# the-byte-bender/GraphAudio

Hardware: AMD Instinct MI355X
Metric: rendered frames/sec @48kHz, 1024-voice convolver graph (higher is better)
Workload: dtype f32

## Files before the change

### graphaudio_amd/csrc/ga_api.cpp

```cpp
#include <algorithm>
#include <cstring>

#include <execinfo.h>
#include <signal.h>
#include <unistd.h>

#include "ga_engine.hpp"

using namespace ga;

static void ga_segv_handler(int sig) {
  void* frames[64];
  int n = backtrace(frames, 64);
  const char msg[] = "\n[graphaudio_hip] fatal signal, native backtrace:\n";
  (void)!write(2, msg, sizeof(msg) - 1);
  backtrace_symbols_fd(frames, n, 2);
  signal(sig, SIG_DFL);
  raise(sig);
}
__attribute__((constructor)) static void ga_install_handler() {
  const char* e = getenv("GA_BACKTRACE");
  if (e && e[0] == '1') signal(SIGSEGV, ga_segv_handler);
}

struct ga_context {
  Context c;
  explicit ga_context(int sr) : c(sr) {}
};

namespace {
template <class F>
int guardRO(ga_context* h, F&& f) {
  if (!h) return GA_ERR_INVALID_ARGUMENT;
  try {
    f(h->c);
    return GA_OK;
  } catch (const Err& e) {
    h->c.lastError = e.msg;
    return e.code;
  } catch (const std::bad_alloc&) {
    h->c.lastError = "out of host memory";
    return GA_ERR_OUT_OF_MEMORY;
  } catch (const std::exception& e) {
    h->c.lastError = e.what();
    return GA_ERR_INVALID_OPERATION;
  } catch (...) {
    h->c.lastError = "unknown error";
    return GA_ERR_INVALID_OPERATION;
  }
}
template <class F>
int guard(ga_context* h, F&& f) {
  if (h) h->c.apiEpoch++;
  return guardRO(h, std::forward<F>(f));
}
NodeS* typed(Context& c, int id, int type) {
  NodeS* n = c.node(id);
  if (n->type != type) fail(GA_ERR_INVALID_ARGUMENT, "node has the wrong type for this call");
  return n;
}
float clampf(float v, float mn, float mx) {
  if (v < mn) return mn;
  if (v > mx) return mx;
  return v;
}
void addEvent(ParamS& p, const ParamEvent& e) {
  size_t lo = 0, hi = p.events.size();
  while (lo < hi) {
    size_t mid = (lo + hi) >> 1;
    if (e.time < p.events[mid].time) hi = mid; else lo = mid + 1;
  }
  p.events.insert(p.events.begin() + lo, e);
}
ParamS makeParam(float def, float mn, float mx, bool arate) {
  ParamS p;
  p.def = def;
  p.minv = mn;
  p.maxv = mx;
  p.arate = arate;
  p.value = def;
  return p;
}
}

int64_t Context::chunkLimit(int64_t) {
    int64_t limit = maxChunkBlocks;
    {
      size_t freeB = 0, totalB = 0;
      if (hipMemGetInfo(&freeB, &totalB) == hipSuccess) {
        double perBlock = 0, fixedBytes = 0;
        int convRowsMax = 0;
        for (auto& g : groups) convRowsMax = std::max(convRowsMax, (int)((g->rows.size() + 127) / 128 * 128));
        perBlock += (double)convRowsMax * kBins * 4.0 * 4.0;
        for (auto& np : nodes)
          if (np->type == GA_NODE_CONVOLVER && np->ir && np->convPath == 4)
          {
            perBlock += (double)((np->isTrueStereo ? 2 : np->ir->nch) + (np->isTrueStereo ? 4 : np->ir->nch)) * 1024.0;
            const double inCh = np->isTrueStereo ? 2 : np->ir->nch, slots = np->isTrueStereo ? 4 : np->ir->nch;
            fixedBytes += (inCh * (np->ir->coarseP + 1) + slots * (double)kCoarseMaxP) * 65536.0;
          }
          else if (np->type == GA_NODE_CONVOLVER && np->ir && np->convPath != 1)
            perBlock += (double)(np->ir->nch + 2 * (np->isTrueStereo ? 2 : np->ir->nch)) * kBins * 8.0;
        perBlock += ((double)nodes.size() * 2.0 + 64.0) * kBlock * 4.0;
        double budget = ((double)freeB + (double)slabBlocks.size() * (double)((size_t)1 << 30) * 0.0) * memBudgetFraction;
        budget += (double)(planes[0].bytes + planes[1].bytes + planes[2].bytes + planes[3].bytes);
        budget += (double)(planesB[0].bytes + planesB[1].bytes + planesB[2].bytes + planesB[3].bytes + planesBalt[0].bytes + planesBalt[1].bytes);
        budget += (double)slabAll.size() * (double)slabFrames * 4.0;
        budget += (double)(coarseX.bytes + coarseY.bytes + coarseM.bytes);
        int64_t byMem = (int64_t)(std::max(budget - fixedBytes, 0.0) / std::max(perBlock, 1.0));
        limit = std::max<int64_t>(1, std::min<int64_t>(limit, byMem));
      }
    }
  return limit;
}

void Context::processBlocks(float* const* outPlanar, float* outInterleaved, int channels, int64_t blockCount, bool deviceOut) {
  if (blockCount < 0) fail(GA_ERR_OUT_OF_RANGE, "blockCount");
  if (disposed) fail(GA_ERR_DISPOSED, "context disposed");
  flushHandOver();
  if (outInterleaved || outPlanar == nullptr) {
    if (channels < 1 || channels > 32) fail(GA_ERR_OUT_OF_RANGE, "channels");
    if (!outInterleaved) fail(GA_ERR_INVALID_ARGUMENT, "Buffer too small for interleaved output.");
  } else if (channels < 0 || channels > 32) {
    fail(GA_ERR_OUT_OF_RANGE, "channels");
  }
  GA_HIP(hipSetDevice(device));
  const hipMemcpyKind kind = deviceOut ? hipMemcpyDeviceToDevice : hipMemcpyDeviceToHost;
  int64_t doneBlocks = 0;
  while (doneBlocks < blockCount) {
    int64_t nblk = std::min(blockCount - doneBlocks, chunkLimit(blockCount - doneBlocks));
    runChunk(nblk, nullptr);
    const int64_t done = chunkBlocksDone;
    if (done <= 0) fail(GA_ERR_INVALID_OPERATION, "render made no progress");
    const int64_t base = doneBlocks * kBlock;
    if (outInterleaved) {
      float* stage = outInterleaved + base * channels;
// ... 10 lines not shown
        stage = ilvDev;
      }
      for (const SegCh& sg : chunkSegCh) {
        InterleaveSrc src{};
        const int used = std::min(channels, sg.ch);
        for (int ch = 0; ch < used; ch++) src.ch[ch] = busSlabs[ch];
        launch_interleave(stream, stage, src, channels, used, sg.b0 * kBlock, (sg.b1 - sg.b0) * kBlock);
      }
      if (!deviceOut)
        GA_HIP(hipMemcpyAsync(outInterleaved + base * channels, ilvDev, (size_t)done * kBlock * channels * sizeof(float), kind, stream));
    } else {
      for (const SegCh& sg : chunkSegCh) {
        const int used = std::min(channels, sg.ch);
        for (int ch = 0; ch < used; ch++)
          if (outPlanar[ch])
            GA_HIP(hipMemcpyAsync(outPlanar[ch] + base + sg.b0 * kBlock, busSlabs[ch] + sg.b0 * kBlock,
                                  sizeof(float) * (size_t)(sg.b1 - sg.b0) * kBlock, kind, stream));
      }
    }
    GA_HIP(hipStreamSynchronize(stream));
    doneBlocks += done;
  }
  stats.device_bytes_in_use = devBytes;
}

void Context::render(float* const* out, int channels, int64_t frameCount, int64_t startIndex, bool deviceOut) {
  if (channels == 0 || !out) fail(GA_ERR_INVALID_ARGUMENT, "Output buffer must have at least one channel.");
  if (frameCount <= 0) fail(GA_ERR_OUT_OF_RANGE, "Frame count must be positive.");
  if (startIndex < 0) fail(GA_ERR_OUT_OF_RANGE, "Start index must be non-negative.");
  if (channels < 0 || channels > 32) fail(GA_ERR_OUT_OF_RANGE, "channelIndex");
  for (int ch = 0; ch < channels; ch++)
    if (!out[ch]) fail(GA_ERR_INVALID_ARGUMENT, "Channel buffer is null.");
  if (disposed) fail(GA_ERR_DISPOSED, "context disposed");
  GA_HIP(hipSetDevice(device));
  const hipMemcpyKind kind = deviceOut ? hipMemcpyDeviceToDevice : hipMemcpyDeviceToHost;
  struct Pipelined {
    Context& c;
    const bool callerAsync;
    explicit Pipelined(Context& cc) : c(cc), callerAsync(cc.asyncMode) { c.asyncMode = true; }
    ~Pipelined() { c.asyncMode = callerAsync; }
  } pipelined(*this);
  struct Drain {
    Context& c;
    const bool blocking;
    ~Drain() {
      if (blocking && c.stream) (void)hipStreamSynchronize(c.stream);
      if (blocking && c.copyStream) (void)hipStreamSynchronize(c.copyStream);
    }
  } drain{*this, !pipelined.callerAsync};
  int64_t written = 0;
  if (cachedFrames > 0) {
    if (channels > cachedCh) fail(GA_ERR_OUT_OF_RANGE, "channelIndex");
    int toCopy = (int)std::min<int64_t>(cachedFrames, frameCount);
    for (int ch = 0; ch < channels; ch++)
      GA_HIP(hipMemcpyAsync(out[ch] + startIndex, cacheDev + (size_t)ch * kBlock + (kBlock - cachedFrames), sizeof(float) * toCopy,
                            kind, stream));
    if (!asyncMode) GA_HIP(hipStreamSynchronize(stream));
    written = toCopy;
    cachedFrames -= toCopy;
  }
  while (written < frameCount) {
    int64_t need = frameCount - written;
    int64_t nblk = (need + kBlock - 1) / kBlock;
    const int64_t limit = chunkLimit(nblk);
    nblk = std::min(nblk, limit);
    bool direct = (deviceOut || hostDirect) && need >= nblk * kBlock;
    float* tgt[32];
    for (int ch = 0; ch < channels && direct; ch++) {
      float* p = out[ch] + startIndex + written;
      if (!deviceOut) {
        hipPointerAttribute_t at{};
        if (hipPointerGetAttributes(&at, p) != hipSuccess || at.type != hipMemoryTypeHost || !at.devicePointer) {
          (void)hipGetLastError();
          direct = false;
          break;
        }
        p = (float*)at.devicePointer;
      }
      tgt[ch] = p;
      direct = (((uintptr_t)p) & 15) == 0;
    }
    struct Target {
      Context& c;
      ~Target() { std::memset(c.busTarget, 0, sizeof(c.busTarget)); }
    } target{*this};
    const bool defer = direct && !deviceOut && pipelined.callerAsync && hostDefer && ownStream;
    if (defer) {
      const size_t rowBytes = ((size_t)nblk * kBlock * sizeof(float) + 255) & ~(size_t)255;
      if (deferStageBytes < rowBytes * 32) {
        flushHandOver();
        if (deferStage) {
          GA_HIP(hipStreamSynchronize(stream));
          dfree(deferStage, deferStageBytes);
        }
        deferStageBytes = rowBytes * 32;
        deferStage = (float*)dalloc(deferStageBytes);
      }
      for (int ch = 0; ch < channels; ch++) busTarget[ch] = (float*)((char*)deferStage + (size_t)ch * (deferStageBytes / 32));
    } else if (direct) {
      for (int ch = 0; ch < channels; ch++) busTarget[ch] = tgt[ch];
    }
    runChunk(nblk, nullptr);
    if (defer)
      for (int ch = 0; ch < channels; ch++)
        pendingHandOver.push_back(HandOver{busTarget[ch], tgt[ch], out[ch] + startIndex + written, chunkBlocksDone * kBlock});
    std::memset(busTarget, 0, sizeof(busTarget));
    const int64_t done = chunkBlocksDone;
    if (done <= 0) fail(GA_ERR_INVALID_OPERATION, "render made no progress");
    if (channels > chunkMinDestCh) fail(GA_ERR_OUT_OF_RANGE, "channelIndex");
    const int64_t chunkFrames = done * kBlock;
    const int64_t toCopy = std::min(chunkFrames, need);
    if (direct) {
    } else if (!deviceOut && ownStream && pipelined.callerAsync && hostCopyStream) {
      handOverToHost(busSlabs.data(), out, channels, startIndex + written, toCopy);
    } else {
      for (int ch = 0; ch < channels; ch++)
        GA_HIP(hipMemcpyAsync(out[ch] + startIndex + written, busSlabs[ch], sizeof(float) * toCopy, kind, stream));
    }
    const int64_t excess = chunkFrames - toCopy;
    if (excess > 0) {
      cachedCh = chunkMinDestCh;
      for (int ch = 0; ch < cachedCh; ch++)
        GA_HIP(hipMemcpyAsync(cacheDev + (size_t)ch * kBlock, busSlabs[ch] + chunkFrames - kBlock, sizeof(float) * kBlock,
                              hipMemcpyDeviceToDevice, stream));
      cachedFrames = (int)excess;
    }
    if (!asyncMode) GA_HIP(hipStreamSynchronize(stream));
    written += toCopy;
  }
  if (!pipelined.callerAsync) {
    GA_HIP(hipStreamSynchronize(stream));
    harvestProfile(true);
  }
  stats.device_bytes_in_use = devBytes;
}

extern "C" {

const char* ga_strerror(int code) {
  switch (code) {
    case GA_OK: return "ok";
    case GA_ERR_INVALID_ARGUMENT: return "invalid argument";
    case GA_ERR_OUT_OF_RANGE: return "argument out of range";
    case GA_ERR_INVALID_OPERATION: return "invalid operation";
    case GA_ERR_DISPOSED: return "object disposed";
    case GA_ERR_CYCLE: return "audio graph cycle detected";
    case GA_ERR_UNSUPPORTED: return "unsupported on the device path";
    case GA_ERR_DEVICE: return "HIP device error";
    case GA_ERR_OUT_OF_MEMORY: return "out of memory";
    case GA_ERR_NO_DEVICE: return "no HIP device";
    default: return "unknown error code";
  }
}
const char* ga_version(void) { return "graphaudio-hip 0.1 (gfx950)"; }
int ga_device_count(void) {
  int n = 0;
  if (hipGetDeviceCount(&n) != hipSuccess) return 0;
  return n;
}

int ga_context_create(int sample_rate, int device_ordinal, ga_context** out) {
  if (!out) return GA_ERR_INVALID_ARGUMENT;
  if (sample_rate <= 0) return GA_ERR_OUT_OF_RANGE;
  ga_context* h = nullptr;
  try {
    h = new ga_context(sample_rate);
    h->c.init_device(device_ordinal);
    auto d = std::make_unique<NodeS>();
    d->id = 0;
    d->type = GA_NODE_DESTINATION;
    d->inputs.resize(1);
    d->inputs[0].channelCount = 2;
    h->c.nodes.push_back(std::move(d));
    *out = h;
    return GA_OK;
  } catch (const Err& e) {
    delete h;
    return e.code;
  } catch (...) {
    delete h;
    return GA_ERR_DEVICE;
  }
}
int ga_context_destroy(ga_context* ctx) {
  delete ctx;
  return GA_OK;
}
const char* ga_last_error(ga_context* ctx) { return ctx ? ctx->c.lastError.c_str() : ""; }
double ga_current_time(ga_context* ctx) { return ctx ? ctx->c.currentTime : 0.0; }
int64_t ga_current_block(ga_context* ctx) { return ctx ? ctx->c.currentBlock : 0; }
int ga_set_option(ga_context* ctx, const char* key, double value) {
  return guard(ctx, [&](Context& c) {
    std::string k = key ? key : "";
    if (k == "max_chunk_blocks") c.maxChunkBlocks = std::max<int64_t>(1, std::min<int64_t>(32768, (int64_t)value));
    else if (k == "profile") c.profile = value != 0;
    else if (k == "profile_every") c.profileEvery = (int)std::max<int64_t>(1, value);
    else if (k == "time_fft") c.useTimeFft = value != 0;
    else if (k == "fft64") c.fft64 = value != 0;
    else if (k == "tconv_radix16") c.useRadix16 = value != 0;
    else if (k == "async") {
      if (c.asyncMode && value == 0) c.synchronize();
      c.asyncMode = value != 0;
    }
    else if (k == "coarse") c.useCoarse = value != 0;
    else if (k == "coarse_overlap") c.coarseOverlap = value != 0;
    else if (k == "coarse_carry") c.coarseCarry = value != 0;
    else if (k == "coarse_tail") c.coarseTail = value != 0;
    else if (k == "coarse_tail_private") c.coarseTailPrivate = value != 0;
    else if (k == "sim_replay") c.simReplay = value != 0;
    else if (k == "twin_channels") c.twinChannels = value != 0;
    else if (k == "cycle_delay_split") c.cycleDelaySplit = value != 0;
    else if (k == "resample_fast") c.resampleFast = value != 0;
    else if (k == "rate_mod_walk") c.rateModWalk = value != 0;
    else if (k == "conv_reference_order") c.convRefOrder = (int)std::min(2.0, std::max(0.0, value));
    else if (k == "conv_ref_min_deviation") c.convRefMinDeviation = std::max(0.0, value);
    else if (k == "coarse_premix") c.coarsePremix = value != 0;
    else if (k == "coarse_ext_history") c.coarseExtHist = value != 0;
    else if (k == "coarse_wide") c.coarseWide = value != 0;
    else if (k == "gain_pass_through") c.gainPassThrough = value != 0;
    else if (k == "gain_fold") c.gainFold = value != 0;
    else if (k == "coarse_mfma") c.coarseMfma = value != 0;
    else if (k == "biquad_time_split") c.biquadTimeSplit = (int)std::min(2.0, std::max(0.0, value));
    else if (k == "biquad_split_max_deviation") c.biquadSplitMaxDeviation = std::max(0.0, value);
    else if (k == "biquad_split_min_frames") c.biquadSplitMinFrames = std::max<int64_t>(2048, (int64_t)value);
    else if (k == "host_direct") c.hostDirect = value != 0;
    else if (k == "host_defer") c.hostDefer = value != 0;
    else if (k == "table_upload_kernel") c.tableUploadKernel = value != 0;
    else if (k == "comm_timeout_s") c.commTimeoutS = std::max(1.0, value);
    else if (k == "host_copy_stream") c.hostCopyStream = value != 0;
    else if (k == "coarse_min_blocks") c.coarseMinBlocks = std::max<int64_t>(1, (int64_t)value);
    else if (k == "debug_tconv_n2") c.debugTconvN2 = (int)value;
    else if (k == "mem_budget_fraction") c.memBudgetFraction = std::min(0.95, std::max(0.05, value));
    else fail(GA_ERR_INVALID_ARGUMENT, "unknown option " + k);
  });
}
int ga_get_stats(ga_context* ctx, ga_stats* out) {
  return guardRO(ctx, [&](Context& c) {
    if (!out) fail(GA_ERR_INVALID_ARGUMENT, "null pointer");
    c.harvestProfile(true);
    c.stats.device_bytes_in_use = c.devBytes;
    c.stats.n_nodes = (int)c.nodes.size();
    int rows = 0;
    for (auto& g : c.groups) rows += (int)g->rows.size();
    c.stats.n_conv_rows = rows;
    *out = c.stats;
  });
}
int ga_synchronize(ga_context* ctx) {
  return guardRO(ctx, [&](Context& c) { c.synchronize(); });
}
int ga_context_set_stream(ga_context* ctx, void* hip_stream) {
  return guard(ctx, [&](Context& c) {
    c.flushHandOver();
    GA_HIP(hipStreamSynchronize(c.stream));
    c.waitHostCopies();
    if (c.ownStream && c.stream) (void)hipStreamDestroy(c.stream);
    c.stream = (hipStream_t)hip_stream;
    c.ownStream = false;
  });
}

int ga_buffer_create(ga_context* ctx, const float* const* planar, int channels, int64_t frames, int sample_rate, int* out_id) {
  return guard(ctx, [&](Context& c) {
    if (!planar || !out_id) fail(GA_ERR_INVALID_ARGUMENT, "null pointer");
    if (channels < 1 || channels > 32) fail(GA_ERR_OUT_OF_RANGE, "Channel count must be between 1 and 32");
    if (frames < 0) fail(GA_ERR_OUT_OF_RANGE, "Length must be non-negative");
    if (sample_rate <= 0) fail(GA_ERR_OUT_OF_RANGE, "Sample rate must be positive");
    auto b = std::make_unique<PlayBuf>();
    b->channels = channels;
    b->length = frames;
    b->sampleRate = sample_rate;
    b->stride = (frames + 8 + 63) / 64 * 64;
    b->host.resize(channels);
    GA_HIP(hipSetDevice(c.device));
    size_t bytes = (size_t)b->stride * channels * sizeof(float);
    b->dev = c.dallocSkewed(bytes, &b->devBase, &b->devBytes);
    GA_HIP(hipMemsetAsync(b->dev, 0, bytes, c.stream));
    for (int i = 0; i < channels; i++) {
      if (!planar[i]) fail(GA_ERR_INVALID_ARGUMENT, "null channel pointer");
      b->host[i].assign(planar[i], planar[i] + frames);
      if (frames)
        GA_HIP(hipMemcpyAsync(b->dev + (size_t)i * b->stride, planar[i], sizeof(float) * frames, hipMemcpyHostToDevice, c.stream));
    }
    GA_HIP(hipStreamSynchronize(c.stream));
    c.buffers.push_back(std::move(b));
    c.bufVersion++;
    *out_id = (int)c.buffers.size() - 1;
  });
}
int ga_buffer_release(ga_context* ctx, int buffer_id) {
  return guard(ctx, [&](Context& c) {
    PlayBuf* b = c.buffer(buffer_id);
    if (!b || b->released) return;
    b->released = true;
    c.releasedPending.push_back(buffer_id);
  });
}

int ga_node_create(ga_context* ctx, int node_type, int* out_id) {
// ... 487 lines not shown
```

### graphaudio_amd/csrc/ga_chunk.cpp

```cpp
#include "ga_chunk_internal.hpp"

namespace ga {

float* getSlab(Context& c) {
  if (c.slabFree.empty()) {
    size_t slabBytes = (size_t)c.slabFrames * sizeof(float);
    size_t count = std::max<size_t>(8, std::min<size_t>(1024, ((size_t)1 << 30) / slabBytes));
    char* blk = (char*)c.dalloc(slabBytes * count);
    c.slabBlocks.push_back(blk);
    for (size_t i = 0; i < count; i++) {
      float* p = (float*)(blk + i * slabBytes);
      c.slabAll.push_back(p);
      c.slabFree.push_back(p);
    }
  }
  float* p = c.slabFree.back();
  c.slabFree.pop_back();
  return p;
}

void resetSlabs(Context& c, int64_t frames) {
  int64_t need = roundup(frames, 256);
  if (need > c.slabFrames) {
    GA_HIP(hipStreamSynchronize(c.stream));
// ... 508 lines not shown
  Context& c_ = *this; (void)c_;
  std::vector<int>& topo = r.topo;
  int& maxDepth = r.maxDepth; int& maxLevel = r.maxLevel; (void)maxDepth; (void)maxLevel;
  int64_t& n = r.n; (void)n;
  std::vector<double>& bt = r.bt; (void)bt;
  std::vector<int>& srcIds = r.srcIds; (void)srcIds;
  std::vector<SrcPlanOut>& srcPlans = r.srcPlans; (void)srcPlans;
  std::vector<Segment>& segs = r.segs; (void)segs;
  const int64_t frames = r.n * kBlock; (void)frames;
  int& bHistMax = r.bHistMax; (void)bHistMax;
  for (int id : topo) {
    NodeS& nd = *nodes[id];
    if (nd.type != GA_NODE_DELAY) continue;
    nd.delayLoaded = false;
    int rings = std::max(nd.delayRings, 2);
    for (const Segment& sg : segs)
      for (const NodeSeg& ns : sg.nodes)
        if (ns.id == id) rings = std::max(rings, ns.ins[0].bufCh);
    nd.delayRings = rings;
    const size_t maxD = (size_t)nd.maxDelaySamples;
    if (nd.delayHistRings < rings) {
      float* nh = (float*)dalloc(maxD * rings * sizeof(float));
      GA_HIP(hipMemsetAsync(nh, 0, maxD * rings * sizeof(float), stream));
      if (nd.delayHist) {
        GA_HIP(hipMemcpyAsync(nh, nd.delayHist, maxD * nd.delayHistRings * sizeof(float), hipMemcpyDeviceToDevice, stream));
        GA_HIP(hipStreamSynchronize(stream));
        dfree(nd.delayHist, maxD * nd.delayHistRings * sizeof(float));
      }
      nd.delayHist = nh;
      nd.delayHistRings = rings;
    }
    const int64_t cap = roundup(frames, 4096);
    if (nd.delayCap < cap || nd.delayLineRings < rings) {
      if (nd.delayLine) {
        GA_HIP(hipStreamSynchronize(stream));
        dfree(nd.delayLine, (maxD + (size_t)nd.delayCap) * nd.delayLineRings * sizeof(float));
      }
      nd.delayCap = std::max(nd.delayCap, cap);
      nd.delayLineRings = rings;
      nd.delayLine = (float*)dalloc((maxD + (size_t)nd.delayCap) * rings * sizeof(float));
    }
    nd.delayW.assign(rings, 0);
    nd.delayR.assign(rings, 0);
  }

  if (r.stage != 2) resetSlabs(*this, frames);
  if (zerosLen < frames) {
    if (zeros) {
      GA_HIP(hipStreamSynchronize(stream));
      dfree(zeros, (size_t)zerosLen * 4);
    }
    zerosLen = roundup(frames, 4096);
    zeros = (float*)dalloc((size_t)zerosLen * 4);
    GA_HIP(hipMemsetAsync(zeros, 0, (size_t)zerosLen * 4, stream));
  }
  if (busCapFrames < frames) {
    GA_HIP(hipStreamSynchronize(stream));
    for (float* p : busSlabs) dfree(p, (size_t)busCapFrames * 4);
    busSlabs.clear();
    busCapFrames = roundup(frames, 4096);
  }
  while ((int)busSlabs.size() < 32 && (int)busSlabs.size() < std::max(destOutCh, 2)) busSlabs.push_back((float*)dalloc((size_t)busCapFrames * 4));
  {
    int mx = 0;
    for (auto& sg : segs)
      if (r.stage != 1) mx = std::max(mx, sg.nodes.back().outCh);
    while ((int)busSlabs.size() < mx) busSlabs.push_back((float*)dalloc((size_t)busCapFrames * 4));
  }

}

void Context::chunkExecute(ChunkRun& r) {
  Context& c_ = *this; (void)c_;
  int& maxDepth = r.maxDepth; int& maxLevel = r.maxLevel; (void)maxDepth; (void)maxLevel;
  int64_t& n = r.n; (void)n;
  std::vector<double>& bt = r.bt; (void)bt;
  std::vector<int>& srcIds = r.srcIds; (void)srcIds;
  std::vector<SrcPlanOut>& srcPlans = r.srcPlans; (void)srcPlans;
  std::vector<Segment>& segs = r.segs; (void)segs;
  const int64_t frames = r.n * kBlock; (void)frames;
  int& bHistMax = r.bHistMax; (void)bHistMax;
  Exec& ex = *r.ex;
  r.tmPlan = nowMs();
  if (!pendingHandOver.empty()) {
    std::vector<HandOver> hv;
    hv.swap(pendingHandOver);
    hipStream_t st = stream;
    ex.plan.launches.insert(ex.plan.launches.begin(), Plan::L{[hv, st](uint8_t*) {
      for (const HandOver& h : hv) GA_HIP(hipMemcpyAsync(h.dst_host, h.src, sizeof(float) * (size_t)h.n, hipMemcpyDeviceToHost, st));
    }, LK_OTHER, 0.0, 0.0});
  }
  ex.trajOffFinal = ex.plan.putv(ex.traj);
  size_t tbytes = ex.plan.host.size();
  const int slot = asyncMode ? (int)(chunkSeq & 1) : 0;
  void*& thost = slot ? tablesHostB : tablesHost;
  size_t& thostBytes = slot ? tablesHostBBytes : tablesHostBytes;
  if (asyncMode && chunkDone[slot]) GA_HIP(hipEventSynchronize(chunkDone[slot]));
  if (thostBytes < tbytes) {
    if (thost) {
      GA_HIP(hipStreamSynchronize(stream));
      (void)hipHostFree(thost);
    }
    thostBytes = (tbytes + tbytes / 4 + 4096 + 15) & ~(size_t)15;
    GA_HIP(hipHostMalloc(&thost, thostBytes, hipHostMallocDefault));
  }
  ensure(tables, std::max(tablesHostBytes, tablesHostBBytes));
  std::memcpy(thost, ex.plan.host.data(), tbytes);
  if (tableUploadKernel) launch_table_upload(stream, tables.p, thost, tbytes);
  else GA_HIP(hipMemcpyAsync(tables.p, thost, tbytes, hipMemcpyHostToDevice, stream));
  uint8_t* base = (uint8_t*)tables.p;

  std::vector<std::pair<hipEvent_t, hipEvent_t>> evs;
  std::vector<int> evKind;
  std::vector<double> evBytes;
  hipEvent_t evBegin = nullptr, evEnd = nullptr;
  const bool profile = profileNow;
  if (profile) {
    GA_HIP(hipEventCreate(&evBegin));
    GA_HIP(hipEventCreate(&evEnd));
    GA_HIP(hipEventRecord(evBegin, stream));
  }
  for (auto& l : ex.plan.launches) {
    hipEvent_t e0 = nullptr, e1 = nullptr;
    if (profile) {
      GA_HIP(hipEventCreate(&e0));
      GA_HIP(hipEventCreate(&e1));
      GA_HIP(hipEventRecord(e0, stream));
    }
    l.fn(base);
    if (profile) {
      GA_HIP(hipEventRecord(e1, stream));
      evs.push_back({e0, e1});
      evKind.push_back(l.kind);
      evBytes.push_back(l.bytes);
    }
    if (l.kind == GA_STAGE_COARSE_SECTION) continue;
    stats.kernel_launches++;
    if (l.kind >= 0 && l.kind < 16) {
      stats.stage_launches[l.kind]++;
      stats.stage_bytes[l.kind] += l.bytes;
      stats.stage_flops[l.kind] += l.flops;
    }
  }
  for (auto& x : extraProf) {
    evs.push_back({x.e0, x.e1});
    evKind.push_back(x.kind);
    evBytes.push_back(x.bytes);
  }
  extraProf.clear();
  if (profile) GA_HIP(hipEventRecord(evEnd, stream));
  GA_HIP(hipGetLastError());
  r.tmLaunch = nowMs();
  if (profileNow) pendingProf.push_back(ProfBatch{evBegin, evEnd, std::move(evs), std::move(evKind), std::move(evBytes)});
  if (asyncMode) {
    if (!chunkDone[slot]) GA_HIP(hipEventCreateWithFlags(&chunkDone[slot], hipEventDisableTiming));
    GA_HIP(hipEventRecord(chunkDone[slot], stream));
    harvestProfile(false);
  } else {
    GA_HIP(hipStreamSynchronize(stream));
    harvestProfile(true);
  }
  chunkSeq++;
  if (gaTiming)
    fprintf(stderr, "[ga]   host detail: topo %.2f, sources %.2f, sim %.2f | resources %.2f, params %.2f, exec %.2f ms\n", r.tmTopo - r.tm0,
            r.tmSrc - r.tmTopo, r.tmSim - r.tmSrc, r.tmRes - r.tmSim, r.tmPre - r.tmRes, r.tmPlan - r.tmPre);
  if (gaTiming)
    fprintf(stderr, "[ga] chunk %lld blocks: sim %.2f ms, plan %.2f ms, enqueue %.2f ms, wait %.2f ms\n", (long long)n, r.tmSim - r.tm0,
            r.tmPlan - r.tmSim, r.tmLaunch - r.tmPlan, nowMs() - r.tmLaunch);

}

void Context::chunkCommit(ChunkRun& r) {
  Context& c_ = *this; (void)c_;
  int& maxDepth = r.maxDepth; int& maxLevel = r.maxLevel; (void)maxDepth; (void)maxLevel;
  int64_t& n = r.n; (void)n;
  std::vector<double>& bt = r.bt; (void)bt;
  std::vector<int>& srcIds = r.srcIds; (void)srcIds;
  std::vector<SrcPlanOut>& srcPlans = r.srcPlans; (void)srcPlans;
  std::vector<Segment>& segs = r.segs; (void)segs;
  const int64_t frames = r.n * kBlock; (void)frames;
  int& bHistMax = r.bHistMax; (void)bHistMax;
  for (size_t i = 0; i < srcIds.size(); i++) {
    NodeS& s = *nodes[srcIds[i]];
    SrcPlanOut& po = srcPlans[i];
    if (s.type != GA_NODE_BUFFER_SOURCE) {
      if (po.gone && po.goneAt <= n) {
        if (!s.endedRaised) endedQueue.push_back(srcIds[i]);
        s.endedRaised = true;
        if (po.goneAt == n) pending.push_back([this, id = srcIds[i]]() { doDispose(id); });
      }
      continue;
    }
    if (s.spans.empty()) continue;
    int64_t firstPlay = -1;
    for (const SrcSpan& sp : s.spans)
      if ((sp.phase == SRC_PLAY || sp.phase == SRC_END) && firstPlay < 0) firstPlay = sp.b0;
    if (firstPlay < 0 || firstPlay >= n) continue;
    int64_t lastProcessed = n;
    if (po.gone && po.goneAt <= n) lastProcessed = po.goneAt;
    int64_t played = lastProcessed - firstPlay;
    PlayBuf* pb = s.bufId >= 0 ? buffers[s.bufId].get() : nullptr;
    bool rate1 = true;
    if (pb) rate1 = sourceGeom(*this, s, *pb).effectiveRate == 1.0;
    if (s.gsr && s.gsrWalked >= 0) {
      if (played == s.gsrWalked) {
        s.playbackPosition = s.gsrTail.pp;
        for (int k = 0; k < 4; k++) s.gsrW[k] = s.gsrTail.w[k];
        s.gsrPos = s.gsrTail.pos;
        s.gsrReady = s.gsrTail.ready;
      } else if (!(po.gone && po.goneAt <= n)) {
        fail(GA_ERR_DEVICE, "internal: a walked source ends its chunk at another block than its walk");
      }
    } else if (s.gsr) {
      if (!s.gsrBlocks.empty()) {
        const GsrBlock& e = s.gsrBlocks[std::min<size_t>((size_t)played, s.gsrBlocks.size() - 1)];
        s.playbackPosition = e.pp;
        for (int k = 0; k < 4; k++) s.gsrW[k] = e.w[k];
        s.gsrPos = e.pos;
        s.gsrReady = e.ready;
      }
    } else if (rate1) {
      s.playbackPosition += played * kBlock;
      if (s.loop && pb) {
        SrcGeom g = sourceGeom(*this, s, *pb);
        int64_t len = g.loopEndFrame - g.loopStartFrame;
        if (s.playbackPosition >= g.loopEndFrame && len > 0)
          s.playbackPosition = g.loopStartFrame + ((s.playbackPosition - g.loopEndFrame) % len);
      }
    } else {
      s.rsBlocks += played;
    }
    if (po.reachedEnd && po.endBlock < n) {
      s.stopTime = bt[po.endBlock + 1];
      s.hasStopped = true;
    }
    if (po.gone && po.goneAt <= n) {
      if (!s.endedRaised) endedQueue.push_back(srcIds[i]);
      s.endedRaised = true;
      if (po.goneAt == n) pending.push_back([this, id = srcIds[i]]() { doDispose(id); });
    }
  }
  for (int id : r.streamIds) streamReplay(*nodes[id], n, bt, true);
  if (r.stage == 1) return;
  currentBlock += n;
  currentTime = bt[n];
  stats.blocks_rendered = currentBlock;
  stats.chunks++;
  stats.segments += (int64_t)segs.size();
  chunkBlocksDone = n;
  chunkSegCh.clear();
  for (const Segment& sg : segs) chunkSegCh.push_back(SegCh{sg.b0, sg.b1, sg.nodes.back().outCh});
}

void Context::runChunkImpl(int64_t nblocks, float* const* ) {
  ChunkRun r;
  r.n = nblocks;
  r.tm0 = nowMs();
  GA_HIP(hipSetDevice(device));
  if (disposed) fail(GA_ERR_DISPOSED, "context disposed");
  drain();
  if (!releasedPending.empty() || ++chunksSinceGc >= 64) collectGarbage();
  latched = true;
  profileNow = profile && (profileSeq++ % std::max(profileEvery, 1)) == 0;
  chunkTopology(r);
  if (!r.rateMods.empty()) {
    runTwoStageChunk(r);
    return;
  }
  chunkSimulate(r);
  chunkResources(r);
  r.tmRes = nowMs();
  bqSplitUsed = 0;
  r.ex = std::make_unique<Exec>(*this, r.n, r.segs);
  r.ex->outViews.resize(r.segs.size());
  r.ex->plan.host.resize(16);
  chunkStaleSeed(r);
  chunkParamCurves(r);
  const double tmPar = nowMs();
  chunkConvScratch(r);
  r.tmPre = nowMs();
  double tmNodes = 0, tmConv = 0;
  for (int d = 0; d <= r.maxDepth; d++) {
    const double a = nowMs();
    chunkPlanNodes(r, d);
    const double b = nowMs();
    chunkPlanConvolvers(r, d);
    tmNodes += b - a;
    tmConv += nowMs() - b;
  }
  chunkDelayCommit(r);
  chunkStaleCommit(r);
  chunkExecute(r);
  const double tmEx = nowMs();
  chunkCommit(r);
  chunkRetire(r);
  if (gaTiming)
    fprintf(stderr, "[ga]   host detail: param curves %.3f, conv scratch %.3f, plan nodes %.3f, plan convolvers %.3f, commit %.3f ms\n",
            tmPar - r.tmRes, r.tmPre - tmPar, tmNodes, tmConv, nowMs() - tmEx);
}

void Context::chunkRetire(ChunkRun& r) {
  if (!r.ex->outViews.empty() && !r.segs.empty()) {
    if (!lastViews.empty() && viewsPool.size() < 8) viewsPool.push_back(std::move(lastViews));
    lastViews = std::move(r.ex->outViews.back());
    r.ex->outViews.pop_back();
    const size_t sl = r.segs.size() - 1;
    if (sl < r.ex->outScale.size() && !r.ex->outScale[sl].empty()) lastViewScale = r.ex->outScale[sl];
    else lastViewScale.clear();
    if (sl < r.ex->outCurve.size() && !r.ex->outCurve[sl].empty()) lastViewCurve = r.ex->outCurve[sl];
    else lastViewCurve.clear();
    lastViewFrames = r.n * kBlock;
    lastViewSlabGen = slabGen;
  }
  for (auto& ov : r.ex->outViews)
    if (!ov.empty() && viewsPool.size() < 8) viewsPool.push_back(std::move(ov));
  if (!r.segs.empty() && simReplay) {
    if (lastSegNodes.capacity() && segNodePool.size() < 8) {
      lastSegNodes.clear();
      segNodePool.push_back(std::move(lastSegNodes));
    }
    lastSegNodes = std::move(r.segs.back().nodes);
    lastSegHash = r.segs.back().hash;
    lastSegEpoch = apiEpoch;
    lastSegGraphVersion = graphVersion;
    r.segs.pop_back();
  }
  for (Segment& sg : r.segs) {
    sg.nodes.clear();
    if (segNodePool.size() < 8) segNodePool.push_back(std::move(sg.nodes));
  }
  r.ex.reset();
}

void Context::runTwoStageChunk(ChunkRun& r) {
  ChunkRun r1;
  r1.stage = 1;
  r1.n = r.n;
  r1.tm0 = r.tm0;
  r1.maxDepth = r.maxDepth;
  r1.maxLevel = r.maxLevel;
  r1.rateMods = r.rateMods;
  r1.coneRoots = std::move(r.coneRoots);
// ... 176 lines not shown
```

### graphaudio_amd/csrc/ga_chunk_internal.hpp

```cpp
#pragma once
#include <time.h>

#include <algorithm>
#include <array>
#include <cstdio>
#include <cstdlib>
#include <cstring>
#include <unordered_map>

#include "ga_engine.hpp"

namespace ga {

static inline uint64_t hmix(uint64_t h, uint64_t v) {
  h ^= v + 0x9e3779b97f4a7c15ull + (h << 6) + (h >> 2);
  return h;
}

static inline int64_t roundup(int64_t v, int64_t m) { return (v + m - 1) / m * m; }

struct Plan {
  std::vector<uint8_t> host;
  struct L {
    std::function<void(uint8_t*)> fn;
// ... 351 lines not shown
        if (!n_.delayAudible && timelineOnly) {
          const ParamS& pd = n_.params[0];
          const double t0 = (*blockTimes)[brel], dts = 1.0 / c.sampleRate;
          bool pending = false;
          for (int r = 0; r < ch && !n_.delayAudible; r++) {
            auto& m = model[r];
            for (auto& run : m.runs)
              if (run.second == OPEN || run.second + maxD >= m.pos) pending = true;
            if (m.runs.empty()) continue;
            for (int i = 0; i < kBlock && !n_.delayAudible; i++) {
              const float dtv = param_value_at(pd.events.data(), (int)pd.events.size(), pd.value, pd.arate ? t0 + i * dts : t0);
              int d = (int)(dtv * (float)c.sampleRate);
              d = std::min(std::max(d, 0), maxD);
              if (d == 0) continue;
              const int64_t q = m.pos + i - d;
              for (auto& run : m.runs)
                if (q >= run.first && (run.second == OPEN || q < run.second)) {
                  n_.delayAudible = true;
                  break;
                }
            }
          }
          if (!n_.delayAudible && pending && extraBreaks) extraBreaks->push_back(brel + 1);
        } else if (!n_.delayAudible && dmax > 0) {
          dmin = std::max(dmin, 1);
          int64_t nextFlip = OPEN;
          for (int r = 0; r < ch && !n_.delayAudible; r++) {
            auto& m = model[r];
            const int64_t lo = m.pos - dmax, hi = m.pos + (kBlock - 1) - dmin;
            for (auto& run : m.runs) {
              const int64_t rs = run.first, re = run.second == OPEN ? OPEN : run.second - 1;
              if (rs <= hi && re >= lo) {
                n_.delayAudible = true;
                break;
              }
              if (rs > hi) {
                int64_t k = (rs + dmin - (kBlock - 1) - m.pos + kBlock - 1) / kBlock;
                nextFlip = std::min(nextFlip, B + std::max<int64_t>(k, 1));
              }
            }
          }
          if (!n_.delayAudible && nextFlip != OPEN && extraBreaks) extraBreaks->push_back(nextFlip - c.currentBlock);
        }
        ns.delayAudible = n_.delayAudible;
        n_.outputs[0].bufCh = ch;
        n_.outputs[0].silent = !n_.delayAudible;
        break;
      }
      default: fail(GA_ERR_UNSUPPORTED, "node type not supported on the device path");
    }
    if (!n_.outputs.empty()) {
      ns.outCh = n_.outputs[0].bufCh;
      ns.outSilent = n_.outputs[0].silent;
      ns.outZero = !n_.outputs[0].silent && n_.outputs[0].zero;
    }
  }

  uint64_t hashSeg(const Segment& s) {
    uint64_t h = 1469598103934665603ull;
    for (const NodeSeg& ns : s.nodes) {
      h = hmix(h, (uint64_t)ns.id);
      h = hmix(h, ((uint64_t)ns.outCh << 8) | (ns.outSilent ? 1 : 0) | ((uint64_t)ns.srcPhase << 4) | (ns.bqActive ? 2 : 0) |
                      ((uint64_t)ns.outMask << 16) | ((uint64_t)ns.panMode << 48) | ((uint64_t)(ns.panDyn ? 1 : 0) << 52) |
                      ((uint64_t)(ns.outZero ? 1 : 0) << 53));
      for (const InSeg& is : ns.ins) {
        h = hmix(h, ((uint64_t)is.bufCh << 1) | (is.silent ? 1 : 0));
        for (const TermS& t : is.terms) h = hmix(h, ((uint64_t)t.node << 16) | ((uint64_t)t.out << 8) | (uint64_t)t.ch | ((uint64_t)t.stale << 60));
      }
      for (const InSeg& is : ns.pins)
        for (const TermS& t : is.terms) h = hmix(h, 0x5151ull ^ (((uint64_t)t.node << 16) | ((uint64_t)t.out << 8) | (uint64_t)t.ch | ((uint64_t)t.stale << 60)));
    }
    for (const InSeg& is : s.probe) {
      h = hmix(h, 0x7070ull ^ (is.silent ? 1 : 0));
      for (const TermS& t : is.terms) h = hmix(h, ((uint64_t)t.node << 16) | ((uint64_t)t.out << 8) | (uint64_t)t.ch);
    }
    return h;
  }
};

struct Exec {
  Context& c;
  int64_t n, frames;
  Plan plan;
  std::vector<Segment>& segs;
  std::unordered_map<uint64_t, float*> nodeSlab, inSlab;
  std::vector<float*> nodeSlab01;
  std::vector<std::vector<Views>> outViews;
  std::vector<const float*> terms;
  std::vector<float> termGains;
  bool anyTermGain = false;
  std::vector<std::vector<float>> outScale;
  float scaleOf(int si, int node) const { return (si < (int)outScale.size() && !outScale[si].empty()) ? outScale[si][node] : 1.f; }
  void setScale(int si, int node, float g) {
    if ((int)outScale.size() <= si) outScale.resize(si + 1);
    if (outScale[si].empty()) outScale[si].assign(c.nodes.size(), 1.f);
    outScale[si][node] = g;
  }
  std::vector<const float*> termCurves;
  bool anyTermCurve = false;
  std::vector<std::vector<const float*>> outCurve;
  const float* curveOf(int si, int node) const { return (si < (int)outCurve.size() && !outCurve[si].empty()) ? outCurve[si][node] : nullptr; }
  void setCurve(int si, int node, const float* cv) {
    if ((int)outCurve.size() <= si) outCurve.resize(si + 1);
    if (outCurve[si].empty()) outCurve[si].assign(c.nodes.size(), nullptr);
    outCurve[si][node] = cv;
  }
  void pushTerm(const float* p, float g, const float* cv = nullptr) {
    termGains.resize(terms.size(), 1.f);
    termCurves.resize(terms.size(), nullptr);
    terms.push_back(p);
    termGains.push_back(g);
    termCurves.push_back(cv);
    if (g != 1.f) anyTermGain = true;
    if (cv) anyTermGain = anyTermCurve = true;
  }
  std::vector<MixJob> mixJobs;
  std::vector<DownmixJob> dmJobs;
  std::vector<GainJob> gainJobs;
  std::vector<BiquadJob> bqJobs[kMaxBiquadSections + 1];
  std::vector<BiquadSection> bqSecs;
  std::vector<BiquadScanJob> bqScans[kMaxBiquadSections + 1];
  std::vector<const std::vector<float>*> bqMats[kMaxBiquadSections + 1];
  int bqG = 0;
  int64_t bqK = 0;
  size_t bqZeroFrom = 0;
  std::vector<BiquadDynJob> bqDynJobs;
  std::vector<LoopJob> loopJobs;
  std::vector<ResampleJob> rsJobs;
  std::vector<ResampleFastJob> rsFastJobs;
  std::vector<GsrJob> gsrJobs;
  std::vector<StreamJob> streamJobs;
  std::vector<ConstJob> constJobs;
  std::vector<OscJob> oscJobs;
  std::vector<PanJob> panJobs;
  std::vector<DelayJob> delayJobs;
  std::vector<PanDynJob> panDynJobs;
  std::vector<ParamModJob> pmodJobs;
  std::vector<ResampleBlock> traj;
  bool mixAligned = true;
  struct ConvInRow {
    Views* p = nullptr;
    size_t n = 0;
    bool empty() const { return n == 0; }
    size_t size() const { return n; }
    Views& operator[](size_t i) const { return p[i]; }
  };
  struct ConvIn {
    std::vector<int> slot;
    std::vector<Views> flat;
    size_t nsegs = 1, used = 0;
    bool has(int id) const { return id < (int)slot.size() && slot[id] >= 0; }
    ConvInRow operator[](int id) {
      if (id >= (int)slot.size()) slot.resize(id + 1, -1);
      if (slot[id] < 0) {
        slot[id] = (int)used++;
        if (flat.size() < used * nsegs) flat.resize(std::max(used * nsegs, 2 * flat.size()));
      }
      return ConvInRow{flat.data() + (size_t)slot[id] * nsegs, nsegs};
    }
  } convIn;

  Exec(Context& c_, int64_t n_, std::vector<Segment>& s) : c(c_), n(n_), frames(n_ * kBlock), segs(s) {
    nodeSlab01.assign(c.nodes.size() * 2, nullptr);
    convIn.slot.assign(c.nodes.size(), -1);
    convIn.nsegs = std::max<size_t>(segs.size(), 1);
  }
// ... 521 lines not shown
```

### graphaudio_amd/csrc/ga_coarse.hip

```cpp
#include "ga_kernels.hpp"
#include "ga_fft16.hpp"

#include <hip/hip_runtime.h>

#include <algorithm>
#include <atomic>
#include <string>
#include <type_traits>
#include <utility>
#include <cstdio>
#include <cstdlib>

namespace ga {

struct LdsLimit {
  std::atomic<uint64_t> done{0};
  void raise(const void* kern, size_t need, const char* what) {
    int dev = 0;
    (void)hipGetDevice(&dev);
    const uint64_t bit = 1ull << (dev & 63);
    if (done.load(std::memory_order_relaxed) & bit) return;
    if (hipFuncSetAttribute(kern, hipFuncAttributeMaxDynamicSharedMemorySize, 160 * 1024) == hipSuccess) {
      done.fetch_or(bit);
      return;
// ... 995 lines not shown
        acc[w].add(x);
      }
    }
  }
}
__global__ __launch_bounds__(64 * kPremixWaves) void coarse_premix_kernel(const PremixJob* __restrict jobs, const PremixTerm* __restrict terms) {
  __shared__ v4f part[kPremixWaves - 1][2][kPremixWords][64];
  const PremixJob J = jobs[blockIdx.y];
  if (J.flags & 4) {
    if (blockIdx.x >= (unsigned)kPremixCopyWgs) return;
    const GA_GLOBAL v4f* src = (const GA_GLOBAL v4f*)terms[J.term0].in;
    GA_GLOBAL v4f* dst = (GA_GLOBAL v4f*)J.out;
    const int64_t nw = J.n / 4, step = (int64_t)kPremixCopyWgs * blockDim.x * 2;
    for (int64_t i = (int64_t)blockIdx.x * blockDim.x * 2 + threadIdx.x; i < nw; i += step) {
      const int64_t i2 = i + blockDim.x;
      const v4f a = src[i], b = i2 < nw ? src[i2] : a;
      dst[i] = a;
      if (i2 < nw) dst[i2] = b;
    }
    return;
  }
  const int64_t tile0 = (int64_t)blockIdx.x * kPremixTile;
  if (tile0 >= J.n) return;
  const int lane = threadIdx.x & 63, wv = __builtin_amdgcn_readfirstlane(threadIdx.x >> 6);
  int64_t f[kPremixWords];
  bool live[kPremixWords], keep[kPremixWords];
  uint32_t off[kPremixWords], coff[kPremixWords];
  Kahan4 acc[kPremixWords];
#pragma unroll
  for (int w = 0; w < kPremixWords; w++) {
    f[w] = tile0 + (int64_t)(w * 64 + lane) * 4;
    live[w] = f[w] < J.n;
    keep[w] = live[w] && f[w] >= J.carry_from;
    off[w] = live[w] ? (uint32_t)(f[w] * 4) : 0u;
    coff[w] = (uint32_t)((f[w] - J.carry_from) * 4);
    acc[w] = Kahan4{v4f{0.f, 0.f, 0.f, 0.f}, v4f{0.f, 0.f, 0.f, 0.f}};
  }
  const int per = ((J.nterms + kPremixWaves - 1) / kPremixWaves + kPremixAhead - 1) / kPremixAhead * kPremixAhead;
  const int t0 = min(J.nterms, wv * per), t1 = min(J.nterms, t0 + per);
  const bool carry_here = (J.flags & 2) && tile0 + kPremixTile > J.carry_from;
  if (J.flags & 1) {
    if (carry_here) premix_stream<true, true>(J, terms, t0, t1, lane, off, keep, coff, acc);
    else premix_stream<true, false>(J, terms, t0, t1, lane, off, keep, coff, acc);
  } else {
    if (carry_here) premix_stream<false, true>(J, terms, t0, t1, lane, off, keep, coff, acc);
    else premix_stream<false, false>(J, terms, t0, t1, lane, off, keep, coff, acc);
  }
  if (wv > 0) {
#pragma unroll
    for (int w = 0; w < kPremixWords; w++) {
      part[wv - 1][0][w][lane] = acc[w].s;
      part[wv - 1][1][w][lane] = acc[w].c;
    }
  }
  __syncthreads();
  if (wv == 0) {
#pragma unroll
    for (int w = 0; w < kPremixWords; w++) {
#pragma unroll
      for (int q = 0; q < kPremixWaves - 1; q++) {
        acc[w].add(part[q][0][w][lane]);
        acc[w].add(-part[q][1][w][lane]);
      }
      if (live[w]) stg4(J.out + f[w], acc[w].s);
    }
  }
}
const char* launch_coarse_premix(hipStream_t s, const PremixJob* jobs_dev, int njobs, const PremixTerm* terms_dev, int64_t max_n) {
  if (njobs <= 0 || max_n <= 0) return "";
  const int64_t gx = (max_n + kPremixTile - 1) / kPremixTile;
  if (gx > 0x7fffffff || max_n >= ((int64_t)1 << 29)) launch_fail("coarse pre-mix: chunk too long");
  for (int j0 = 0; j0 < njobs; j0 += 32768)
    hipLaunchKernelGGL(coarse_premix_kernel, dim3((unsigned)gx, std::min(32768, njobs - j0)), dim3(64 * kPremixWaves), 0, s, jobs_dev + j0, terms_dev);
  return "coarse_premix_kernel";
}

void launch_coarse_hist(hipStream_t s, const CoarseHistJob* jobs_dev, int njobs, int64_t max_len) {
  if (njobs <= 0 || max_len <= 0) return;
  const int gx = (int)std::min<int64_t>((max_len / 4 + 255) / 256, 64);
  for (int j0 = 0; j0 < njobs; j0 += 32768)
    hipLaunchKernelGGL(coarse_hist_kernel, dim3(gx, std::min(32768, njobs - j0)), dim3(256), 0, s, jobs_dev + j0);
}

__global__ __launch_bounds__(256) void table_upload_kernel(v4f* __restrict dst, const v4f* __restrict src, size_t n16) {
  for (size_t i = (size_t)blockIdx.x * 256 + threadIdx.x; i < n16; i += (size_t)gridDim.x * 256) ((GA_GLOBAL v4f*)dst)[i] = ((const GA_GLOBAL v4f*)src)[i];
}
void launch_table_upload(hipStream_t s, void* dst, const void* src_pinned, size_t bytes) {
  const size_t n16 = (bytes + 15) / 16;
  if (!n16) return;
  const unsigned grid = (unsigned)std::min<size_t>((n16 + 255) / 256, 64);
  hipLaunchKernelGGL(table_upload_kernel, dim3(grid), dim3(256), 0, s, (v4f*)dst, (const v4f*)src_pinned, n16);
}

}
```

### graphaudio_amd/csrc/ga_comm.cpp

```cpp
#include <dlfcn.h>

#include <cstring>
#include <mutex>

#include <chrono>
#include <thread>

#include "ga_engine.hpp"

#if __has_include(<rccl/rccl.h>)
#include <rccl/rccl.h>
static_assert(NCCL_UNIQUE_ID_BYTES == GA_COMM_ID_BYTES, "include/graphaudio_hip.h: GA_COMM_ID_BYTES != NCCL_UNIQUE_ID_BYTES");
static_assert(sizeof(ncclUniqueId) == GA_COMM_ID_BYTES, "ncclUniqueId is passed by value as GA_COMM_ID_BYTES bytes");
static_assert((int)ncclSuccess == 0 && (int)ncclInProgress == 7, "restated ncclResult_t values");
static_assert((int)ncclFloat32 == 7 && (int)ncclSum == 0, "restated ncclDataType_t / ncclRedOp_t values");
#endif

namespace ga {

namespace {
constexpr int kNcclSuccess = 0, kNcclInProgress = 7, kNcclFloat32 = 7, kNcclSum = 0;
struct UniqueId {
  char internal[GA_COMM_ID_BYTES];
};
// ... 108 lines not shown
    if (r.CommGetAsyncError && r.CommGetAsyncError(comm, &async) == kNcclSuccess && async != kNcclSuccess && async != kNcclInProgress) {
      const std::string what = r.GetErrorString ? r.GetErrorString(async) : "RCCL error";
      commAbort();
      fail(GA_ERR_DEVICE, "the communicator failed (a peer rank aborted or died): " + what);
    }
    if (std::chrono::duration<double>(std::chrono::steady_clock::now() - t0).count() > commTimeoutS) {
      commAbort();
      fail(GA_ERR_DEVICE, "timed out waiting for the sharded render's collective (option comm_timeout_s)");
    }
    std::this_thread::sleep_for(std::chrono::microseconds(200));
  }
}

void Context::commDestroy() {
  if (comm) {
    try {
      if (stream) commWait();
    } catch (...) {
    }
  }
  if (comm) {
    Rccl& r = rccl();
    if (r.CommDestroy) (void)r.CommDestroy(comm);
    comm = nullptr;
  }
  commDead = false;
  commRanks = 0;
  commRank = 0;
  if (reduceBuf) {
    dfree(reduceBuf, reduceBytes);
    reduceBuf = nullptr;
    reduceBytes = 0;
  }
}

void Context::renderReduce(float* const* out, int channels, int64_t frames, int64_t start, int root) {
  if (commRanks < 1) fail(GA_ERR_INVALID_OPERATION, "ga_comm_init has not been called on this context");
  if (commDead) fail(GA_ERR_INVALID_OPERATION, "the communicator was aborted after an error; ga_comm_destroy and ga_comm_init again");
  if (root < 0 || root >= commRanks) fail(GA_ERR_OUT_OF_RANGE, "root");
  if (channels < 1 || channels > 32) fail(GA_ERR_OUT_OF_RANGE, "channelIndex");
  if (frames <= 0) fail(GA_ERR_OUT_OF_RANGE, "Frame count must be positive.");
  if (start < 0) fail(GA_ERR_OUT_OF_RANGE, "Start index must be non-negative.");
  const bool isRoot = commRank == root;
  if (isRoot) {
    if (!out) fail(GA_ERR_INVALID_ARGUMENT, "Output buffer must have at least one channel.");
    for (int ch = 0; ch < channels; ch++)
      if (!out[ch]) fail(GA_ERR_INVALID_ARGUMENT, "Channel buffer is null.");
  }
  GA_HIP(hipSetDevice(device));
  const size_t need_ = (size_t)channels * (size_t)frames * sizeof(float);
  if (reduceBytes < need_) {
    flushHandOver();
    if (reduceBuf) {
      GA_HIP(hipStreamSynchronize(stream));
      dfree(reduceBuf, reduceBytes);
    }
    reduceBytes = need_ + need_ / 8;
    reduceBuf = (float*)dalloc(reduceBytes);
  }
  float* rows[32];
  for (int ch = 0; ch < channels; ch++) rows[ch] = reduceBuf + (size_t)ch * frames;
  const bool callerAsync = asyncMode;
  asyncMode = true;
  try {
    render(rows, channels, frames, 0, true);
    if (comm) {
      Rccl& r = rccl();
      check(r, r.Reduce(reduceBuf, reduceBuf, (size_t)channels * frames, kNcclFloat32, kNcclSum, root, comm, stream), "ncclReduce");
    }
    if (isRoot) {
      float* devAlias[32];
      bool locked = callerAsync && hostDefer && ownStream && (frames % 4) == 0;
      for (int ch = 0; ch < channels && locked; ch++) {
        hipPointerAttribute_t at{};
        if (hipPointerGetAttributes(&at, out[ch] + start) != hipSuccess || at.type != hipMemoryTypeHost || !at.devicePointer ||
            (((uintptr_t)at.devicePointer) & 15)) {
          (void)hipGetLastError();
          locked = false;
        } else {
          devAlias[ch] = (float*)at.devicePointer;
        }
      }
      if (locked) {
        for (int ch = 0; ch < channels; ch++) pendingHandOver.push_back(HandOver{rows[ch], devAlias[ch], out[ch] + start, frames});
      } else if (callerAsync && ownStream && hostCopyStream) {
        handOverToHost(rows, out, channels, start, frames);
      } else {
        for (int ch = 0; ch < channels; ch++)
          GA_HIP(hipMemcpyAsync(out[ch] + start, rows[ch], (size_t)frames * sizeof(float), hipMemcpyDeviceToHost, stream));
      }
    }
  } catch (...) {
    asyncMode = callerAsync;
    commAbort();
    throw;
  }
  asyncMode = callerAsync;
  if (!callerAsync) {
    flushHandOver();
    commWait();
    harvestProfile(true);
  }
}

}
```

### graphaudio_amd/csrc/ga_engine.cpp

```cpp
#include "ga_engine.hpp"

#include <algorithm>
#include <cstdio>
#include <cstring>

namespace ga {

void launch_fail(const char* what) { fail(GA_ERR_INVALID_OPERATION, std::string("internal: ") + what); }

void* Context::dalloc(size_t bytes) {
  void* p = nullptr;
  if (bytes == 0) bytes = 256;
  GA_HIP(hipMalloc(&p, bytes));
  devBytes += (int64_t)bytes;
  return p;
}
float* Context::dallocSkewed(size_t bytes, void** base, size_t* total) {
  *total = bytes + 64 * 1024;
  *base = dalloc(*total);
  return (float*)((char*)*base + (size_t)(skewSeq++ % 64) * 1024);
}
double Context::biquadDeviation(const float* coefs, int nsec) {
  std::vector<float> key(coefs, coefs + 5 * nsec);
  uint64_t h = 1469598103934665603ull;
// ... 111 lines not shown
  float* p = (float*)((char*)bqSplitBlocks[blk] + bqSplitUsed % kBqSplitBlock);
  bqSplitUsed += bytes;
  return p;
}
int Context::persistentBuffer(const float* p, int64_t n) {
  if (!p || n <= 0) return -1;
  if (bufSpansVersion != bufVersion) {
    bufSpans.clear();
    for (size_t i = 0; i < buffers.size(); i++)
      if (buffers[i] && buffers[i]->dev) bufSpans.push_back(BufSpan{buffers[i]->dev, buffers[i]->dev + (size_t)buffers[i]->stride * buffers[i]->channels, (int)i});
    std::sort(bufSpans.begin(), bufSpans.end(), [](const BufSpan& a, const BufSpan& b) { return a.lo < b.lo; });
    bufSpansVersion = bufVersion;
  }
  auto it = std::upper_bound(bufSpans.begin(), bufSpans.end(), p, [](const float* q, const BufSpan& s) { return q < s.lo; });
  if (it == bufSpans.begin()) return -1;
  --it;
  return (p >= it->lo && p + n <= it->hi) ? it->id : -1;
}
void Context::dfree(void* p, size_t bytes) {
  if (!p) return;
  (void)hipFree(p);
  devBytes -= (int64_t)(bytes == 0 ? 256 : bytes);
}
void Context::ensure(DevArena& a, size_t bytes) {
  if (a.bytes >= bytes) return;
  if (a.p) {
    GA_HIP(hipStreamSynchronize(stream));
    dfree(a.p, a.bytes);
    a.p = nullptr;
    a.bytes = 0;
  }
  size_t nb = bytes + bytes / 8;
  a.p = dalloc(nb);
  a.bytes = nb;
  GA_HIP(hipMemsetAsync(a.p, 0, nb, stream));
}

void Context::init_device(int dev) {
  int count = 0;
  if (hipGetDeviceCount(&count) != hipSuccess || count <= 0)
    fail(GA_ERR_NO_DEVICE, "no HIP device visible: libgraphaudio_hip has no CPU fallback");
  if (dev < 0 || dev >= count) fail(GA_ERR_INVALID_ARGUMENT, "device ordinal out of range");
  device = dev;
  GA_HIP(hipSetDevice(dev));
  GA_HIP(hipStreamCreateWithFlags(&stream, hipStreamNonBlocking));
  ownStream = true;
  const double pi = 3.14159265358979323846264338327950288;
  std::vector<double2> t128(64), t256(129);
  for (int j = 0; j < 64; j++) t128[j] = make_double2(std::cos(2.0 * pi * j / 128.0), -std::sin(2.0 * pi * j / 128.0));
  for (int k = 0; k <= 128; k++) t256[k] = make_double2(std::cos(2.0 * pi * k / 256.0), -std::sin(2.0 * pi * k / 256.0));
  w128 = (double2*)dalloc(sizeof(double2) * 64);
  w256 = (double2*)dalloc(sizeof(double2) * 129);
  GA_HIP(hipMemcpy(w128, t128.data(), sizeof(double2) * 64, hipMemcpyHostToDevice));
  GA_HIP(hipMemcpy(w256, t256.data(), sizeof(double2) * 129, hipMemcpyHostToDevice));
  cacheDev = (float*)dalloc(sizeof(float) * 32 * kBlock);
}

Context::~Context() {
  if (stream) (void)hipStreamSynchronize(stream);
  try {
    commDestroy();
  } catch (...) {
  }
  for (auto& b : buffers)
    if (b && b->devBase) (void)hipFree(b->devBase);
  for (auto& g : groups) {
    if (g->histR) (void)hipFree(g->histR);
    if (g->histI) (void)hipFree(g->histI);
    if (g->overlap[0]) (void)hipFree(g->overlap[0]);
    if (g->overlap[1]) (void)hipFree(g->overlap[1]);
  }
  for (auto& a : planes)
    if (a.p) (void)hipFree(a.p);
  for (auto& a : planesB)
    if (a.p) (void)hipFree(a.p);
  for (auto& a : planesBalt)
    if (a.p) (void)hipFree(a.p);
  for (auto& np : nodes) {
    if (np && np->bHistR) (void)hipFree(np->bHistR);
    if (np && np->bHistI) (void)hipFree(np->bHistI);
    if (np && np->bOverlap) (void)hipFree(np->bOverlap);
    if (np && np->dHistBase[0]) (void)hipFree(np->dHistBase[0]);
    if (np && np->dHistBase[1]) (void)hipFree(np->dHistBase[1]);
    if (np && np->dTail[0]) (void)hipFree(np->dTail[0]);
    if (np && np->dTail[1]) (void)hipFree(np->dTail[1]);
    if (np && np->stWin[0]) (void)hipFree(np->stWin[0]);
    if (np && np->stWin[1]) (void)hipFree(np->stWin[1]);
    if (np && np->delayHist) (void)hipFree(np->delayHist);
    if (np && np->delayLine) (void)hipFree(np->delayLine);
    if (np && np->oscPhase) (void)hipFree(np->oscPhase);
    if (np && np->panDev) (void)hipFree(np->panDev);
  }
  for (auto& kv : tw16) (void)hipFree(kv.second);
  if (rateModDev) (void)hipFree(rateModDev);
  if (rateModHost) (void)hipHostFree(rateModHost);
  if (coarseTw) (void)hipFree(coarseTw);
  if (tw16pw) (void)hipFree(tw16pw);
  if (copyStream) {
    (void)hipStreamSynchronize(copyStream);
    (void)hipStreamDestroy(copyStream);
    for (int k = 0; k < 2; k++) {
      if (outReady[k]) (void)hipEventDestroy(outReady[k]);
      if (outCopied[k]) (void)hipEventDestroy(outCopied[k]);
      if (outStage[k]) (void)hipFree(outStage[k]);
    }
  }
  if (stream2) {
    (void)hipStreamSynchronize(stream2);
    (void)hipStreamDestroy(stream2);
    for (auto& e : dGroupEv)
      if (e) (void)hipEventDestroy(e);
    if (dJoinEv) (void)hipEventDestroy(dJoinEv);
  }
  for (auto& x : extraProf) { (void)hipEventDestroy(x.e0); (void)hipEventDestroy(x.e1); }
  if (coarseX.p) (void)hipFree(coarseX.p);
  if (coarseY.p) (void)hipFree(coarseY.p);
  if (coarseM.p) (void)hipFree(coarseM.p);
  if (deferStage) (void)hipFree(deferStage);
  for (auto& r : retired) (void)hipFree(r.first);
  for (auto& kv : resamplers)
    if (kv.second->devSamples) (void)hipFree(kv.second->devSamples);
  for (auto& np : nodes)
    if (np && np->staleBuf) {
      (void)hipFree(np->staleBuf);
      (void)hipFree(np->staleNext);
    }
  for (float* p : bqSplitBlocks) (void)hipFree(p);
  if (ilvDev) (void)hipFree(ilvDev);
  if (tables.p) (void)hipFree(tables.p);
  if (tablesHost) (void)hipHostFree(tablesHost);
  if (tablesHostB) (void)hipHostFree(tablesHostB);
  for (auto& e : chunkDone)
    if (e) (void)hipEventDestroy(e);
  for (auto& b : pendingProf) {
    (void)hipEventDestroy(b.begin);
    (void)hipEventDestroy(b.end);
    for (auto& e : b.evs) { (void)hipEventDestroy(e.first); (void)hipEventDestroy(e.second); }
  }
  for (void* p : slabBlocks) (void)hipFree(p);
  for (void* p : bqBlocks) (void)hipFree(p);
  for (float* p : busSlabs) (void)hipFree(p);
  if (zeros) (void)hipFree(zeros);
  if (w128) (void)hipFree(w128);
  if (w256) (void)hipFree(w256);
  for (auto& kv : twC) (void)hipFree(kv.second);
  if (cacheDev) (void)hipFree(cacheDev);
  if (stream && ownStream) (void)hipStreamDestroy(stream);
}

void Context::executeOrPost(std::function<void()> cmd) {
  if (disposed) fail(GA_ERR_DISPOSED, "context disposed");
  if (latched && !inRender) cmd(); else pending.push_back(std::move(cmd));
}
void Context::post(std::function<void()> cmd) {
  if (disposed) fail(GA_ERR_DISPOSED, "context disposed");
  pending.push_back(std::move(cmd));
}
void Context::drain() {
  while (!pending.empty()) {
    auto cmd = std::move(pending.front());
    pending.pop_front();
    apiEpoch++;
    try {
      cmd();
    } catch (const Err&) {
    }
  }
}

NodeS* Context::node(int id) {
  if (id < 0 || id >= (int)nodes.size()) fail(GA_ERR_INVALID_ARGUMENT, "bad node id");
  return nodes[id].get();
}
ParamS* Context::param(int nid, int p) {
  NodeS* n = node(nid);
  if (p < 0 || p >= (int)n->params.size()) fail(GA_ERR_INVALID_ARGUMENT, "bad param index");
  return &n->params[p];
}
PlayBuf* Context::buffer(int id) {
  if (id < 0) return nullptr;
  if (id >= (int)buffers.size() || !buffers[id]) fail(GA_ERR_INVALID_ARGUMENT, "bad buffer id");
  return buffers[id].get();
}
void Context::collectGarbage() {
  chunksSinceGc = 0;
  if (!releasedPending.empty()) {
    std::vector<char> used(buffers.size(), 0);
    for (auto& np : nodes) {
      if (!np || np->disposed) continue;
      if (np->bufId >= 0 && np->bufId < (int)used.size()) used[np->bufId] = 1;
      if (np->irBuf >= 0 && np->irBuf < (int)used.size()) used[np->irBuf] = 1;
      for (auto& e : np->dHistExt)
        if (e.first && e.second >= 0 && e.second < (int)used.size()) used[e.second] = 1;
      if (np->type == GA_NODE_STREAM_SOURCE) {
        if (np->stCurrent >= 0 && np->stCurrent < (int)used.size()) used[np->stCurrent] = 1;
        for (int id : np->stQueued) if (id >= 0 && id < (int)used.size()) used[id] = 1;
        for (int id : np->stProcessed) if (id >= 0 && id < (int)used.size()) used[id] = 1;
      }
    }
    std::vector<int> keep;
    bool synced = false;
    for (int id : releasedPending) {
      if (id < 0 || id >= (int)buffers.size() || !buffers[id]) continue;
      if (used[id]) {
        keep.push_back(id);
        continue;
      }
      if (!synced && stream) {
        (void)hipStreamSynchronize(stream);
        synced = true;
      }
      PlayBuf& b = *buffers[id];
      if (b.devBase) dfree(b.devBase, b.devBytes);
      bufVersion++;
      for (auto it = irCache.begin(); it != irCache.end();)
        it = it->first.first == id ? irCache.erase(it) : std::next(it);
      buffers[id].reset();
    }
    releasedPending.swap(keep);
  }
  for (auto it = irCache.begin(); it != irCache.end();) {
    if (it->second.use_count() == 1) {
      if (stream) (void)hipStreamSynchronize(stream);
      it = irCache.erase(it);
    } else {
      ++it;
    }
  }
}

InputS* Context::inputOf(const InRef& r) {
  NodeS* n = nodes[r.node].get();
  if (r.input >= 0) return &n->inputs[r.input];
  return nullptr;
}

void Context::harvestProfile(bool wait) {
  while (!pendingProf.empty()) {
    ProfBatch& b = pendingProf.front();
    if (wait) GA_HIP(hipEventSynchronize(b.end));
    else if (hipEventQuery(b.end) != hipSuccess) { (void)hipGetLastError(); break; }
    float ms = 0;
    GA_HIP(hipEventElapsedTime(&ms, b.begin, b.end));
    stats.device_ms_total += ms;
    stats.profiled_chunks++;
    for (size_t i = 0; i < b.evs.size(); i++) {
      GA_HIP(hipEventElapsedTime(&ms, b.evs[i].first, b.evs[i].second));
      const int k = b.kinds[i];
      if (k == LK_MAC || k == LK_CMAC) stats.mac_ms_total += ms;
      else if (k == LK_FFT || k == LK_IFFT || k == LK_CFWD || k == LK_CINV || k == LK_CHIST) stats.fft_ms_total += ms;
      else if (k != GA_STAGE_COARSE_SECTION) stats.other_ms_total += ms;
      if (k >= 0 && k < 16) stats.stage_ms[k] += ms;
      (void)hipEventDestroy(b.evs[i].first);
      (void)hipEventDestroy(b.evs[i].second);
    }
    (void)hipEventDestroy(b.begin);
    (void)hipEventDestroy(b.end);
    pendingProf.pop_front();
  }
}
void Context::flushHandOver() {
  for (const HandOver& h : pendingHandOver)
    GA_HIP(hipMemcpyAsync(h.dst_host, h.src, sizeof(float) * (size_t)h.n, hipMemcpyDeviceToHost, stream));
  pendingHandOver.clear();
}
void Context::synchronize() {
  GA_HIP(hipSetDevice(device));
  flushHandOver();
  commWait();
  waitHostCopies();
  harvestProfile(true);
  freeRetired();
}
void Context::freeRetired() {
  for (auto& r : retired) dfree(r.first, r.second);
  retired.clear();
}
void Context::waitHostCopies() {
  if (!copyStream) return;
  GA_HIP(hipStreamSynchronize(copyStream));
  outPending[0] = outPending[1] = false;
}
void Context::handOverToHost(const float* const* src, float* const* out, int channels, int64_t offset, int64_t frames) {
  if (!copyStream) {
    GA_HIP(hipStreamCreateWithFlags(&copyStream, hipStreamNonBlocking));
    for (int k = 0; k < 2; k++) {
      GA_HIP(hipEventCreateWithFlags(&outReady[k], hipEventDisableTiming));
      GA_HIP(hipEventCreateWithFlags(&outCopied[k], hipEventDisableTiming));
    }
  }
  const int k = outCur;
  outCur ^= 1;
  const size_t need = (size_t)channels * (size_t)frames * sizeof(float);
  if (outStageBytes[k] < need) {
    if (outPending[k]) GA_HIP(hipEventSynchronize(outCopied[k]));
    outPending[k] = false;
    if (outStage[k]) {
      GA_HIP(hipStreamSynchronize(stream));
      dfree(outStage[k], outStageBytes[k]);
      outStage[k] = nullptr;
      outStageBytes[k] = 0;
    }
    outStage[k] = (float*)dalloc(need);
    outStageBytes[k] = need;
  }
  if (outPending[k]) GA_HIP(hipStreamWaitEvent(stream, outCopied[k], 0));
  for (int ch = 0; ch < channels; ch++)
    GA_HIP(hipMemcpyAsync(outStage[k] + (size_t)ch * frames, src[ch], sizeof(float) * (size_t)frames, hipMemcpyDeviceToDevice, stream));
  GA_HIP(hipEventRecord(outReady[k], stream));
  GA_HIP(hipStreamWaitEvent(copyStream, outReady[k], 0));
  for (int ch = 0; ch < channels; ch++)
    GA_HIP(hipMemcpyAsync(out[ch] + offset, outStage[k] + (size_t)ch * frames, sizeof(float) * (size_t)frames, hipMemcpyDeviceToHost, copyStream));
  GA_HIP(hipEventRecord(outCopied[k], copyStream));
  outPending[k] = true;
}

void Context::connectTo(int src, int out, InRef in) {
  graphVersion++;
  if (in.node == src) fail(GA_ERR_INVALID_OPERATION, "Cannot connect a node to itself");
  OutputS& o = nodes[src]->outputs[out];
  if (std::find(o.connectedInputs.begin(), o.connectedInputs.end(), in) != o.connectedInputs.end()) return;
  o.connectedInputs.push_back(in);
  if (in.input >= 0) {
    InputS& i = nodes[in.node]->inputs[in.input];
    Conn c{src, out};
    if (std::find(i.connected.begin(), i.connected.end(), c) == i.connected.end()) {
      i.connected.push_back(c);
      i.dirty = true;
    }
  } else {
    auto& m = nodes[in.node]->params[-1 - in.input].modulation;
    std::pair<int, int> c{src, out};
    if (std::find(m.begin(), m.end(), c) == m.end()) m.push_back(c);
  }
}
static void removeFromInput(Context& c, int src, int out, InRef in) {
  if (in.input >= 0) {
    InputS& i = c.nodes[in.node]->inputs[in.input];
    Conn cc{src, out};
    auto it = std::find(i.connected.begin(), i.connected.end(), cc);
    if (it != i.connected.end()) i.connected.erase(it);
    i.dirty = true;
  } else {
    auto& m = c.nodes[in.node]->params[-1 - in.input].modulation;
// ... 11 lines not shown
    removeFromInput(*this, src, out, in);
  }
}
void Context::outputDisconnectAll(int src, int out) {
  graphVersion++;
  OutputS& o = nodes[src]->outputs[out];
  std::vector<InRef> ins = o.connectedInputs;
  o.connectedInputs.clear();
  for (const InRef& in : ins) removeFromInput(*this, src, out, in);
}
void Context::inputDisconnectAll(InRef in) {
  std::vector<Conn> outs;
  if (in.input >= 0) {
    outs = nodes[in.node]->inputs[in.input].connected;
  } else {
    for (auto& m : nodes[in.node]->params[-1 - in.input].modulation) outs.push_back(Conn{m.first, m.second});
  }
  for (const Conn& c : outs) disconnectFrom(c.node, c.out, in);
  if (in.input >= 0) nodes[in.node]->inputs[in.input].dirty = true;
}
void Context::doDispose(int id) {
  graphVersion++;
  NodeS& n = *nodes[id];
  if (n.disposed) return;
  n.disposed = true;
  for (int o = 0; o < (int)n.outputs.size(); o++) outputDisconnectAll(id, o);
  for (int i = 0; i < (int)n.inputs.size(); i++) {
    inputDisconnectAll(InRef{id, i});
    n.inputs[i].bufCh = 0;
  }
  for (int p = 0; p < (int)n.params.size(); p++) inputDisconnectAll(InRef{id, -1 - p});
  if (n.type == GA_NODE_DELAY) {
    if (stream) (void)hipStreamSynchronize(stream);
    if (n.delayHist) dfree(n.delayHist, (size_t)n.maxDelaySamples * n.delayHistRings * sizeof(float));
    if (n.delayLine) dfree(n.delayLine, ((size_t)n.maxDelaySamples + (size_t)n.delayCap) * n.delayLineRings * sizeof(float));
    n.delayHist = n.delayLine = nullptr;
    n.delayHistRings = n.delayLineRings = 0;
    n.delayCap = 0;
  }
  if (n.staleBuf) {
    if (stream) (void)hipStreamSynchronize(stream);
    dfree(n.staleBuf, (size_t)n.staleRows * kBlock * sizeof(float));
    dfree(n.staleNext, (size_t)n.staleRows * kBlock * sizeof(float));
    n.staleBuf = n.staleNext = nullptr;
    n.staleRows = 0;
  }
  if (n.type == GA_NODE_BUFFER_SOURCE) n.bufId = -1;
  if (n.type == GA_NODE_STREAM_SOURCE && n.stState != GA_STREAM_STOPPED) {
    n.stState = GA_STREAM_STOPPED;
    streamFlushToProcessed(n);
  }
  if (n.type == GA_NODE_CONVOLVER) {
    releaseConvState(n);
    n.ir.reset();
    n.irBuf = -1;
  }
}

void Context::releaseConvState(NodeS& n) {
  graphVersion++;
  for (auto& r : n.convRows)
    if (r.group) r.group->rows[r.idx] = {-1, 0};
  n.convRows.clear();
  if (n.bHistR || n.bOverlap) {
    if (stream) (void)hipStreamSynchronize(stream);
    if (n.ir) {
      size_t hb = (size_t)n.bInCh * kBins * std::max(n.ir->P - 1, 1) * sizeof(float);
      dfree(n.bHistR, hb);
      dfree(n.bHistI, hb);
    } else {
      (void)hipFree(n.bHistR);
      (void)hipFree(n.bHistI);
    }
    dfree(n.bOverlap, (size_t)n.bSlots * 2 * kBlock * sizeof(float));
  }
  if (n.dHist[0]) {
    if (stream) (void)hipStreamSynchronize(stream);
    dfree(n.dHistBase[0], n.dHistBytes);
    dfree(n.dHistBase[1], n.dHistBytes);
    n.dHistBase[0] = n.dHistBase[1] = nullptr;
  }
  if (n.dTail[0]) {
    if (stream) (void)hipStreamSynchronize(stream);
    for (int b = 0; b < 2; b++) dfree(n.dTail[b], (size_t)n.dTailLen * n.dTailCh * sizeof(float));
  }
  n.dTail[0] = n.dTail[1] = nullptr;
  n.dTailLen = 0;
  n.dTailCh = n.dTailCur = 0;
  n.dTailSig = 0;
  n.dTailSeq = ~0ull - 1;
  n.dHist[0] = n.dHist[1] = nullptr;
  n.dHistExt.clear();
  n.dHistLen = 0;
  n.dHistCur = 0;
  n.dHistZero = true;
  n.dLeader = -1;
  n.dGroupSize = 0;
  n.everFed = false;
  fusionKeyValid = false;
  n.bHistR = n.bHistI = n.bOverlap = nullptr;
  n.bHistPlane = -1;
  n.convPath = 0;
  n.bShared = true;
  n.bHistZero = true;
  n.bOvCur = 0;
}

void Context::flushPlaneHistories(int pair) {
  std::vector<HistJobB> jobs;
  int maxh = 1;
  for (int id : bResidents[pair]) {
    NodeS* n = node(id);
    if (!n || n->bHistPlane != pair || !n->ir || !n->bHistR) continue;
    const int h = n->ir->P - 1;
    const size_t hstride = (size_t)kBins * std::max(h, 1);
    for (int c = 0; c < n->bHistNx && h > 0; c++) {
      const size_t off = (size_t)(n->bHistRow + c) * kBins * n->bHistTxb + n->bHistOff;
      jobs.push_back(HistJobB{n->bHistR + c * hstride, xPlane(pair, 0) + off, h, n->bHistTxb, h, 0});
      jobs.push_back(HistJobB{n->bHistI + c * hstride, xPlane(pair, 1) + off, h, n->bHistTxb, h, 0});
    }
    maxh = std::max(maxh, h);
    n->bHistPlane = -1;
  }
  bResidents[pair].clear();
  if (jobs.empty()) return;
  HistJobB* tab = nullptr;
  GA_HIP(hipHostMalloc((void**)&tab, jobs.size() * sizeof(HistJobB), hipHostMallocDefault));
  memcpy(tab, jobs.data(), jobs.size() * sizeof(HistJobB));
  launch_hist_copy_b(stream, tab, (int)jobs.size(), maxh);
  GA_HIP(hipGetLastError());
  GA_HIP(hipStreamSynchronize(stream));
  GA_HIP(hipHostFree(tab));
}

ConvRowRef Context::addGroupRow(const std::shared_ptr<IrSpectra>& ir, int ch, int depth, int nodeId) {
  auto key = std::make_tuple(ir.get(), ch, depth);
  ConvGroup* g;
  auto it = groupOf.find(key);
  if (it == groupOf.end()) {
    auto ng = std::make_unique<ConvGroup>();
    ng->ir = ir;
    ng->irCh = ch;
    ng->depth = depth;
    ng->P = ir->P;
    g = ng.get();
    groups.push_back(std::move(ng));
    groupOf[key] = g;
  } else {
    g = it->second;
  }
  int idx = (int)g->rows.size();
  g->rows.push_back({nodeId, ch});
  if (idx < g->rp && g->histR) {
    const int hist = g->P - 1;
    if (hist > 0) {
      GA_HIP(hipMemset2DAsync(g->histR + idx, (size_t)g->rp * 4, 0, 4, (size_t)kBins * hist, stream));
      GA_HIP(hipMemset2DAsync(g->histI + idx, (size_t)g->rp * 4, 0, 4, (size_t)kBins * hist, stream));
    }
    GA_HIP(hipMemsetAsync(g->overlap[0] + (size_t)idx * kBlock, 0, kBlock * 4, stream));
    GA_HIP(hipMemsetAsync(g->overlap[1] + (size_t)idx * kBlock, 0, kBlock * 4, stream));
  }
  return ConvRowRef{g, idx};
}

void Context::refOrderSensitivity(const std::vector<int>& topo) {
  bool anyConv = false;
  for (int id : topo) anyConv = anyConv || (nodes[id]->type == GA_NODE_CONVOLVER && nodes[id]->ir);
  if (!anyConv) return;
  if (convRefOrder != 1) {
// ... 475 lines not shown
```

### graphaudio_amd/csrc/ga_engine.hpp

```cpp
#pragma once
#include <cstring>
#include <initializer_list>
#include <new>
#include <hip/hip_runtime.h>

#include <algorithm>
#include <cmath>
#include <cstdint>
#include <deque>
#include <functional>
#include <limits>
#include <map>
#include <tuple>
#include <memory>
#include <string>
#include <unordered_map>
#include <vector>

#include "../../include/graphaudio_hip.h"
#include "ga_kernels.hpp"
#include "ga_gsr.hpp"

namespace ga {

// ... 119 lines not shown
  double offset = 0, duration = std::numeric_limits<double>::infinity();
  int64_t playbackPosition = 0;
  bool loop = false;
  double loopStart = 0, loopEnd = 0;
  int64_t rsBlocks = 0;
  int64_t rsStartPos = 0;
  std::vector<SrcSpan> spans;
  bool gsr = false;
  double rsRate = 0.0;
  int rsBufId = -1;
  int rsChannels = 0;
  int64_t gsrW[4] = {-1, -1, -1, -1};
  double gsrPos = 0.0;
  int gsrReady = 0;
  std::vector<GsrBlock> gsrBlocks;
  uint64_t gsrDevOff = 0;
  bool gsrUploaded = false;
  const GsrBlock* gsrDesc = nullptr;
  int64_t gsrWalked = -1;
  GsrBlock gsrTail{};
  int oscType = 0;
  double* oscPhase = nullptr;
  bool oscPhaseReset = false;
  int64_t schedLo = 0, schedHi = 0;
  float panLast = std::nanf(""), panGL = 0.5f, panGR = 0.5f;
  PanState* panDev = nullptr;
  bool panOnDevice = false;
  uint64_t bqDynSeq = ~0ull, panDynSeq = ~0ull;
  bool bqDynChunk_unused = false;
  bool panDynChunk_unused = false;
  int maxDelaySamples = 0;
  int delayCh = 0;
  int delayRings = 0;
  bool delayAudible = false;
  float* delayHist = nullptr;
  int delayHistRings = 0;
  float* delayLine = nullptr;
  int64_t delayCap = 0;
  int delayLineRings = 0;
  std::vector<int64_t> delayR;
  std::vector<int64_t> delayW;
  bool delayLoaded = false;
  struct DelayRingModel {
    int64_t pos = 0;
    bool open = false;
    std::vector<std::pair<int64_t, int64_t>> runs;
  };
  std::vector<DelayRingModel> delayModel;
  int64_t delayPrevEval = -1;
  int delayPrevCh = 0;
  int filterType = GA_FILTER_LOWPASS;
  float b0 = 0, b1 = 0, b2 = 0, a1 = 0, a2 = 0;
  bool coefDirty = true;
  bool coefMemoValid = false;
  int coefMemoType = -1;
  float coefMemoIn[3] = {0, 0, 0}, coefMemoOut[5] = {0, 0, 0, 0, 0};
  BiquadDynState* bqDyn = nullptr;
  float* bqState = nullptr;
  int bqTwinN = 32;
  bool coefOnDevice = false;
  int irBuf = -1;
  std::shared_ptr<IrSpectra> ir;
  int effectiveOutCh = 0;
  bool isTrueStereo = false, normalize = true, enableTrueStereo = true;
  std::vector<ConvRowRef> convRows;
  int convPath = 0;
  int bInCh = 0, bSlots = 0;
  float* bHistR = nullptr;
  float* bHistI = nullptr;
  float* bOverlap = nullptr;
  int bOvCur = 0;
  bool bShared = true;
  int bHistPlane = -1;
  int bHistRow = 0, bHistNx = 1, bHistOff = 0, bHistTxb = 0;
  bool bHistZero = true;
  std::vector<std::pair<const float*, int>> dHistExt;
  float* dHist[2] = {nullptr, nullptr};
  void* dHistBase[2] = {nullptr, nullptr};
  size_t dHistBytes = 0;
  int64_t dHistLen = 0;
  int dHistCur = 0;
  bool dHistZero = true;
  bool everFed = false;
  float* dTail[2] = {nullptr, nullptr};
  int64_t dTailLen = 0;
  int dTailCh = 0, dTailCur = 0;
  uint64_t dTailSig = 0, dTailSeq = ~0ull - 1;
  std::deque<int> stQueued, stProcessed;
  int stCurrent = -1;
  int64_t stPos = 0;
  int stLastRate = 0;
  const float* stRateMod = nullptr;
  int stState = GA_STREAM_STOPPED;
  int stChannels = -1;
  double stRsPos = 0.0;
  int stRsReady = 0;
  bool stWinValid = false;
  float* stWin[2] = {nullptr, nullptr};
  int stWinCur = 0;
  struct StreamBlockInfo { int outCh; bool silent; };
  std::vector<StreamBlockInfo> stInfo;
  std::vector<StreamBlock> stBlocks;
  std::vector<StreamPiece> stPieces;
  std::vector<StreamSeg> stSegs;
  int64_t stWend[4] = {0, 0, 0, 0};
  int stWendSeg[4] = {-1, -1, -1, -1};
  bool stFed = false;
  uint64_t stBlocksOff = 0, stPiecesOff = 0, stSegsOff = 0;
  bool stUploaded = false;
  int dLeader = -1;
  int dGroupSize = 0;
  bool refSens = false, refOrder = false;
  bool staleProducer = false;
  bool delaySplit = false;
  float* staleBuf = nullptr;
  float* staleNext = nullptr;
  int staleRows = 0;
  uint64_t staleSeq = 0;
};

template <class T, int N>
class SmallVec {
 public:
  SmallVec() {}
  explicit SmallVec(size_t n) { resize(n); }
  SmallVec(size_t n, const T& v) { assign(n, v); }
  SmallVec(std::initializer_list<T> il) { for (const T& v : il) push_back(v); }
  SmallVec(const SmallVec& o) { for (const T& v : o) push_back(v); }
  SmallVec(SmallVec&& o) noexcept { take(std::move(o)); }
  ~SmallVec() { clear(); release(); }
  SmallVec& operator=(const SmallVec& o) {
    if (this != &o) { clear(); reserve(o.n_); for (const T& v : o) push_back(v); }
    return *this;
  }
  SmallVec& operator=(SmallVec&& o) noexcept {
    if (this != &o) { clear(); release(); take(std::move(o)); }
    return *this;
  }
  size_t size() const { return n_; }
  bool empty() const { return n_ == 0; }
  T* data() { return p_; }
  const T* data() const { return p_; }
  T& operator[](size_t i) { return p_[i]; }
  const T& operator[](size_t i) const { return p_[i]; }
  T* begin() { return p_; }
  T* end() { return p_ + n_; }
  const T* begin() const { return p_; }
  const T* end() const { return p_ + n_; }
  T& front() { return p_[0]; }
  const T& front() const { return p_[0]; }
  T& back() { return p_[n_ - 1]; }
  const T& back() const { return p_[n_ - 1]; }
  void clear() {
    for (size_t i = 0; i < n_; i++) p_[i].~T();
    n_ = 0;
  }
  void reserve(size_t c) {
    if (c <= cap_) return;
    size_t nc = std::max<size_t>(c, 2 * cap_);
    T* np = static_cast<T*>(::operator new(nc * sizeof(T)));
    for (size_t i = 0; i < n_; i++) {
      new (np + i) T(std::move(p_[i]));
      p_[i].~T();
    }
    release();
    p_ = np;
    cap_ = nc;
// ... 119 lines not shown
enum LaunchKind { LK_OTHER = GA_STAGE_OTHER, LK_MIX = GA_STAGE_MIX, LK_FFT = GA_STAGE_RFFT_FWD, LK_MAC = GA_STAGE_MAC,
                  LK_IFFT = GA_STAGE_RFFT_INV, LK_CFWD = GA_STAGE_COARSE_FWD, LK_CMAC = GA_STAGE_COARSE_MAC,
                  LK_CINV = GA_STAGE_COARSE_INV, LK_CHIST = GA_STAGE_COARSE_HIST, LK_CPREMIX = GA_STAGE_COARSE_PREMIX };

struct DevArena {
  void* p = nullptr;
  size_t bytes = 0;
};

struct Resampler {
  double rate = 1.0;
  std::vector<ResampleBlock> blocks;
  int64_t consumedEnd = 0;
  double posEnd = 0.0;
  int readyEnd = 0;
  int devOffset = -1;
  std::vector<ResampleSample> pending;
  ResampleSample* devSamples = nullptr;
  int64_t devBlocks = 0, devCapBlocks = 0;
  bool samplesOk = true;
  void extend(int64_t nblocks);
};

struct ChunkRun;
struct Exec;
struct NodePlanCtx;
struct ConvPlanCtx;

void biquadCoefficients(int filterType, float sampleRate, float frequency, float q, float gain, float o[5]);

struct Context {
  int sampleRate;
  int device = 0;
  hipStream_t stream = nullptr;
  bool ownStream = true;
  int64_t currentBlock = 0;
  double currentTime = 0.0;
  bool disposed = false;
  bool latched = false;
  bool inRender = false;
  std::deque<std::function<void()>> pending;
  std::vector<std::unique_ptr<NodeS>> nodes;
  std::vector<std::unique_ptr<PlayBuf>> buffers;
  std::map<std::pair<int, int>, std::shared_ptr<IrSpectra>> irCache;
  std::vector<std::unique_ptr<ConvGroup>> groups;
  std::map<std::tuple<IrSpectra*, int, int>, ConvGroup*> groupOf;
  std::map<uint64_t, std::unique_ptr<Resampler>> resamplers;
  std::string lastError;
  ga_stats stats{};
  int64_t maxChunkBlocks = 4096;
  double memBudgetFraction = 0.7;
  bool profile = false;
  int profileEvery = 1;
  int64_t profileSeq = 0;
  bool profileNow = false;
  double2* w128 = nullptr;
  double2* w256 = nullptr;
  std::map<int, float2*> twC;
  float* zeros = nullptr;
  int64_t zerosLen = 0;
  DevArena planes[4];
  DevArena planesB[4];
  DevArena planesBalt[2];
  int bPairCur = 0;
  int bPairWrite = 0;
  size_t bRowX = 0, bRowY = 0;
  std::vector<int> bResidents[2];
  float* xPlane(int pair, int im) { return (float*)(pair == 0 ? planesB[im].p : planesBalt[im].p); }
  void flushPlaneHistories(int pair);
  DevArena tables;
  bool tableUploadKernel = true;
  void* tablesHost = nullptr;
  size_t tablesHostBytes = 0;
  bool asyncMode = false;
  void* tablesHostB = nullptr;
  size_t tablesHostBBytes = 0;
  uint64_t chunkSeq = 0;
  hipEvent_t chunkDone[2] = {nullptr, nullptr};
  struct ProfBatch {
    hipEvent_t begin, end;
    std::vector<std::pair<hipEvent_t, hipEvent_t>> evs;
    std::vector<int> kinds;
    std::vector<double> bytes;
  };
  std::deque<ProfBatch> pendingProf;
  void harvestProfile(bool wait);
  void synchronize();
  std::vector<float*> slabFree, slabAll;
  int64_t slabFrames = 0;
  std::vector<void*> slabBlocks;
  std::vector<void*> bqBlocks;
  size_t bqUsed = 0;
  int64_t devBytes = 0;
  int destOutCh = 0;
  float* cacheDev = nullptr;
  int cachedFrames = 0, cachedCh = 0;

  explicit Context(int sr) : sampleRate(sr) {}
  ~Context();
  void init_device(int device);
  void* dalloc(size_t bytes);
  void dfree(void* p, size_t bytes);
  void ensure(DevArena& a, size_t bytes);
  float* dallocSkewed(size_t bytes, void** base, size_t* total);
  int persistentBuffer(const float* p, int64_t n);
  struct BufSpan { const float* lo; const float* hi; int id; };
  std::vector<BufSpan> bufSpans;
  uint64_t bufVersion = 1, bufSpansVersion = 0;
  bool coarseExtHist = true;
  bool coarseMfma = true;
  bool coarseWide = true;
  bool gainFold = true;
  bool gainPassThrough = true;
  int biquadTimeSplit = 1;
  int64_t biquadSplitMinFrames = 16384;
  struct BqTransition { std::vector<float> key; std::vector<float> M; };
  std::unordered_map<uint64_t, std::vector<std::pair<std::vector<float>, double>>> bqDeviations;
  double biquadDeviation(const float* coefs, int nsec);
  std::unordered_map<uint64_t, std::vector<BqTransition>> bqTransitions;
  const BqTransition& biquadTransition(const float* coefs, int nsec, int64_t K);
  double biquadSplitMaxDeviation = 2.5e-6;
  std::vector<float*> bqSplitBlocks;
  size_t bqSplitUsed = 0;
  static constexpr size_t kBqSplitBlock = (size_t)4 << 20;
  float* bqSplitAlloc(size_t floats);
  unsigned skewSeq = 0;

  void executeOrPost(std::function<void()> cmd);
  void post(std::function<void()> cmd);
  void drain();

  NodeS* node(int id);
  ParamS* param(int node, int p);
  PlayBuf* buffer(int id);
  std::vector<int> releasedPending;
  int64_t chunksSinceGc = 0;
  void collectGarbage();
  InputS* inputOf(const InRef& r);

  void connectTo(int src, int out, InRef in);
  void disconnectFrom(int src, int out, InRef in);
  void outputDisconnectAll(int src, int out);
  void inputDisconnectAll(InRef in);
  void doDispose(int id);

  std::shared_ptr<IrSpectra> irSpectra(int bufId, bool normalize);
  void releaseConvState(NodeS& n);
  void refOrderSensitivity(const std::vector<int>& topo);
  bool ensureResampleSamples(Exec& ex, Resampler& rs, int64_t upto);
  bool rateModWalk = true;
  bool resampleFast = true;
  void assignConvPaths(const std::vector<int>& topo, int64_t chunkBlocks);
  hipStream_t copyStream = nullptr;
  bool hostCopyStream = false;
  hipEvent_t outReady[2] = {nullptr, nullptr}, outCopied[2] = {nullptr, nullptr};
  float* outStage[2] = {nullptr, nullptr};
  size_t outStageBytes[2] = {0, 0};
  bool outPending[2] = {false, false};
  int outCur = 0;
  void handOverToHost(const float* const* src, float* const* out, int channels, int64_t offset, int64_t frames);
  void waitHostCopies();
  hipStream_t stream2 = nullptr;
  hipEvent_t dGroupEv[8] = {nullptr, nullptr, nullptr, nullptr, nullptr, nullptr, nullptr, nullptr};
  hipEvent_t dJoinEv = nullptr;
  bool coarseOverlap = false;
  bool coarseTail = true;
// ... 16 lines not shown
  DevArena coarseX, coarseY;
  float2* coarseTw = nullptr;
  const float2* coarseTwab();
  float2* tw16pw = nullptr;
  const float2* twiddles16pw();
  void ensureCoarseSpectra(IrSpectra& ir);
  void planCoarseFusion(const std::vector<int>& topo, const std::vector<Segment>& segs);
  uint64_t fusionKey = 0;
  bool fusionKeyValid = false;
  void aliasBusToLeader(ChunkRun& r);
  ConvRowRef addGroupRow(const std::shared_ptr<IrSpectra>& ir, int ch, int depth, int nodeId);
  void ensureGroupState(ConvGroup& g);
  const float2* twiddlesC(int N2);
  const float2* twiddles16(int N2);
  std::map<int, float2*> tw16;
  bool useRadix16 = true;
  bool useCoarse = true;
  int64_t coarseMinBlocks = 256;
  int debugTconvN2 = 0;
  const float2* ensureTapSpectra(IrSpectra& ir, int N2);
  struct TconvLaunch { int N2, tbase, nseg; };
  std::vector<TconvLaunch> tconvPlan(int nblocks, int P) const;
  bool fft64 = false;
  bool useTimeFft = true;
  void updateBiquadCoefficients(NodeS& n, float frequency, float q, float gain);

  void render(float* const* out, int channels, int64_t frames, int64_t start, bool deviceOut);
  void runChunk(int64_t nblocks, float* const* bus);
  void runChunkImpl(int64_t nblocks, float* const* bus);
  void chunkTopology(ChunkRun& r);
  void chunkSimulate(ChunkRun& r);
  void chunkResources(ChunkRun& r);
  void chunkParamCurves(ChunkRun& r);
  void chunkConvScratch(ChunkRun& r);
  void chunkPlanNodes(ChunkRun& r, int depth);
  void planConstantSource(NodePlanCtx& k);
  void planOscillator(NodePlanCtx& k);
  void planDelay(NodePlanCtx& k);
  void planStereoPanner(NodePlanCtx& k);
  void planBufferSource(NodePlanCtx& k);
  void planStreamSource(NodePlanCtx& k);
  void planGain(NodePlanCtx& k);
  void planBiquad(NodePlanCtx& k);
  void chunkPlanConvolvers(ChunkRun& r, int depth);
  void planConvolversShared(ChunkRun& r, int depth, ConvPlanCtx& k);
  void planConvolversPrivate(ChunkRun& r, int depth, ConvPlanCtx& k, bool refOrder);
  void chunkDelayCommit(ChunkRun& r);
  void chunkStaleSeed(ChunkRun& r);
  void chunkStaleCommit(ChunkRun& r);
  void chunkExecute(ChunkRun& r);
  void chunkCommit(ChunkRun& r);
  void chunkRetire(ChunkRun& r);
  void runTwoStageChunk(ChunkRun& r);
  void chunkRateProbe(ChunkRun& r);
  std::vector<std::pair<int, int>> topoRateMods;
  std::vector<char> rateCone;
  uint64_t rateModsVersion = ~0ull;
  void* rateModDev = nullptr;
  size_t rateModDevBytes = 0;
  void* rateModHost = nullptr;
  size_t rateModHostBytes = 0;
  void ensureBiquadState(NodeS& bn);
  void streamReplay(NodeS& s, int64_t nblocks, const std::vector<double>& bt, bool commit);
  void streamFlushToProcessed(NodeS& s);
  bool faulted = false;
  std::string faultMsg;
  int chunkPhase = 0;

  void* comm = nullptr;
  int commRanks = 0, commRank = 0;
  float* reduceBuf = nullptr;
  size_t reduceBytes = 0;
  bool commDead = false;
  double commTimeoutS = 120.0;
  void commInit(const void* id, int nRanks, int rank);
  void commDestroy();
  void commInfo(int* nRanks, int* rank, int* usesRccl);
  void commAbort();
  void commWait();
  void renderReduce(float* const* out, int channels, int64_t frames, int64_t start, int root);

  int64_t busCapFrames = 0;
  std::vector<float*> busSlabs;
  struct HandOver { const float* src; float* dst_dev; float* dst_host; int64_t n; };
  std::vector<HandOver> pendingHandOver;
  std::vector<std::pair<void*, size_t>> retired;
  void freeRetired();
  float* deferStage = nullptr;
  size_t deferStageBytes = 0;
  bool hostDefer = true;
  void flushHandOver();
  float* busTarget[32] = {};
  bool hostDirect = true;
  struct SegCh { int64_t b0, b1; int ch; };
  std::vector<SegCh> chunkSegCh;
  float* ilvDev = nullptr;
  size_t ilvBytes = 0;
  void processBlocks(float* const* outPlanar, float* outInterleaved, int channels, int64_t blockCount, bool deviceOut);
  int64_t chunkLimit(int64_t nblk);
  std::vector<uint32_t> fuseStamp;
  std::vector<const NodeSeg*> fuseSeg;
  std::vector<int> fuseAbs, fuseLen;
  uint32_t fuseEpoch = 0;
  uint64_t graphVersion = 1, topoVersion = 0;
  std::vector<int> topoCache;
  int topoMaxDepth = 0, topoMaxLevel = 0;
  std::deque<int> endedQueue;
  uint64_t lastHash = 0;
  std::vector<NodeSeg> lastSegNodes;
  uint64_t lastSegHash = 0, lastSegEpoch = 0, lastSegGraphVersion = 0;
  bool lastSegStable = false;
  uint64_t apiEpoch = 0;
  bool simReplay = true;
  bool twinChannels = true;
  bool topoHasTimeNodes = false, topoHasConvolvers = false, topoHasOscillators = false, topoHasStreams = false;
  bool topoHasCycles = false;
  std::vector<int> staleProducers;
  std::vector<int> staleLeavers;
  double loopGainBound = 0.0;
  std::vector<int> topoRefOrder;
  std::vector<std::pair<int, int>> topoRefEntry;
  int cycleBlocks = 1;
  bool cycleDelaySplit = true;
  std::vector<Views> lastViews;
  std::vector<float> lastViewScale;
  std::vector<const float*> lastViewCurve;
  int64_t lastViewFrames = 0;
  uint64_t slabGen = 0, lastViewSlabGen = ~0ull;
  uint64_t topoStatsVersion = ~0ull;
  size_t topoStatsSize = 0;
  std::vector<std::pair<int, int>> curveList;
  uint64_t curveListEpoch = ~0ull, curveListGraphVersion = ~0ull;
  size_t curveListTopoSize = 0;
  std::vector<int> deviceStateNodes;
  int chunkMinDestCh = 0;
  int64_t chunkBlocksDone = 0;
};

void commUniqueId(void* out);

}
```

### graphaudio_amd/csrc/ga_kernels.hpp

```cpp
#pragma once
#include <hip/hip_runtime.h>
#include <stdint.h>
#include <stdlib.h>

namespace ga {

[[noreturn]] void launch_fail(const char* what);

#ifdef GA_EXPERIMENTS
inline const char* expenv(const char* name) { return getenv(name); }
#else
inline const char* expenv(const char*) { return nullptr; }
#endif

constexpr int kBlock = 128;
constexpr int kBins = 129;

struct ConvPlanes {
  float* xr;
  float* xi;
  float* yr;
  float* yi;
  int tx;
  int ty;
// ... 64 lines not shown
void launch_tconv(hipStream_t s, const ConvSetC* sets_dev, int nsets, int nblocks, int hist, ConvPlanesB pl, int N2, const float2* tw,
                  int nseg);
void launch_tconv16(hipStream_t s, const ConvSetC* sets_dev, int nsets, int nblocks, int hist, ConvPlanesB pl, int N2, const float2* tw16,
                    int nseg, int tbase);

constexpr int kCoarseBlock = 8192;
constexpr int kCoarseMaxP = 16;
constexpr int kCoarseJobTerms = 32;
constexpr int kCoarseSumJobBlocks(int columns) { return columns <= 2 ? 72 : 40; }
#ifndef GA_MAC_TW4
#define GA_MAC_TW4 4
#endif
constexpr int kCoarseJobBlocks(int columns) { return columns <= 2 ? 72 : (columns == 16 ? 32 : 8 * GA_MAC_TW4); }
constexpr double kCoarseTransformFlops = 2.0 * 3.0 * 256.0 * 200.0 + 2048.0 * 60.0;
constexpr int kCoarseBins = 8192;
struct CoarseXRow {
  const float* hist;
  const float* in;
  int64_t nvalid;
  int frame0;
  int n_frames;
  int u0;
  int hist_len;
  int flags;
  float scale;
  float* carry;
  int64_t carry_from;
};
struct CoarseHandOver {
  const float* src;
  float* dst;
  int64_t n;
};
struct CoarseTerm {
  int frame0;
  int pad_;
  const float2* h[16];
};
struct CoarseJob {
  int term0, n_terms;
  int P;
  int t0, n_t;
  int yrow0;
  int shared_h;
  int u_lo, u_hi;
  int pad_;
};
struct CoarseOut {
  float* out;
  int64_t nvalid;
  int y0, ny;
  const float* tail_in;
  float* tail_out;
  int64_t tail_len;
  int n_y;
  int pad_;
};
struct CoarseHistJob {
  const float* old_hist;
  const float* in;
  float* new_hist;
  int64_t hist_len, n;
};
struct PremixTerm {
  const float* in;
  float* carry;
};
struct PremixJob {
  float* out;
  int term0, nterms;
  int64_t n;
  int64_t carry_from;
  int flags;
  int pad_;
};
const char* launch_coarse_premix(hipStream_t s, const PremixJob* jobs_dev, int njobs, const PremixTerm* terms_dev, int64_t max_n);
const char* launch_coarse_fwd(hipStream_t s, const CoarseXRow* rows_dev, int nrows, int max_frames, int run, float2* X, const float2* tw16,
                       const float2* twab, const CoarseHandOver* handover_dev = nullptr, int n_handover = 0);
const char* launch_coarse_mac(hipStream_t s, const CoarseJob* jobs_dev, int njobs, const CoarseTerm* terms_dev, const float2* X, float2* Y,
                       int y_frames, int cw, int max_t, int maxP, bool any_private, int pb, bool matrix_cores = false);
const char* launch_coarse_inv(hipStream_t s, const CoarseOut* outs_dev, int nouts, int n_t, const int* ylist_dev, const float2* Y, int y_frames,
                       const float2* tw16, const float2* twab);
void launch_coarse_hist(hipStream_t s, const CoarseHistJob* jobs_dev, int njobs, int64_t max_len);
void launch_table_upload(hipStream_t s, void* dst, const void* src_pinned, size_t bytes);

struct MixJob {
  float* out;
  int term0;
  int nterms;
  int64_t f0;
  int64_t n;
  float* out2 = nullptr;
};
void launch_mix(hipStream_t s, const MixJob* jobs_dev, int njobs, const float* const* terms_dev, int64_t max_n, bool vec4, const float* gains_dev = nullptr,
                const float* const* curves_dev = nullptr);

void launch_mix_wide(hipStream_t s, const MixJob* jobs_dev, int njobs, const float* const* terms_dev, int64_t max_n, const float* gains_dev = nullptr,
                     const float* const* curves_dev = nullptr);
constexpr int kMixWideMinTerms = 256;

struct DownmixJob {
  float* out;
  int term0;
  int nch;
  float scale;
  int64_t f0;
  int64_t n;
};
void launch_downmix(hipStream_t s, const DownmixJob* jobs_dev, int njobs, const float* const* terms_dev, int64_t max_n, const float* gains_dev = nullptr);

struct GainJob {
  const float* in;
  float* out;
  const float* curve;
  const float* mod;
  float gain;
  float vmin, vmax;
  int64_t f0;
  int64_t n;
};
void launch_gain(hipStream_t s, const GainJob* jobs_dev, int njobs, int64_t max_n);

constexpr int kMaxBiquadSections = 8;
struct BiquadSection {
  float b0, b1, b2, a1, a2;
  float pad_;
  float* state;
};
struct BiquadJob {
  const float* in;
  float* out;
  int sec0;
  int nsec;
  int64_t f0;
  int64_t n;
  float* state;
  int twins = 1;
  int pad_ = 0;
};
void launch_biquad(hipStream_t s, const BiquadJob* jobs_dev, int njobs, const BiquadSection* secs_dev, int nsec);

struct BiquadScanJob {
  const float* in;
  float* out;
  uint64_t m_off;
  float* scratch;
  int sec0, nsec;
  int64_t f0, n;
  int twins = 1;
  int pad_ = 0;
};
void launch_biquad_split_expand(hipStream_t s, const BiquadScanJob* casc_dev, int ncasc, int G, int64_t K, BiquadJob* passA, BiquadJob* passB);
void launch_biquad_lanes(hipStream_t s, const BiquadJob* jobs_dev, int njobs, const BiquadSection* secs_dev, int nsec, bool state_only = false);
void launch_biquad_scan(hipStream_t s, const BiquadScanJob* casc_dev, int ncasc, int G, const BiquadSection* secs_dev, const uint8_t* tables, int nsec = 0);

struct BiquadDynState {
  float b0, b1, b2, a1, a2;
  int dirty;
  float w[64];
};
struct BiquadDynJob {
  const float* in[32];
  float* out[32];
  const float* fcurve;
  const float* qcurve;
  const float* gcurve;
// ... 249 lines not shown
```

### graphaudio_amd/csrc/ga_plan_conv.cpp

```cpp
#include "ga_chunk_internal.hpp"

namespace ga {

void Context::ensureGroupState(ConvGroup& g) {
  Context& c = *this;
  int need = (int)roundup(std::max<size_t>(g.rows.size(), 1), 128);
  if (need <= g.rp) return;
  const int hist = g.P - 1;
  size_t hBytes = (size_t)kBins * std::max(hist, 1) * need * sizeof(float);
  size_t oBytes = (size_t)need * kBlock * sizeof(float);
  float* nr = (float*)c.dalloc(hBytes);
  float* ni = (float*)c.dalloc(hBytes);
  float* o0 = (float*)c.dalloc(oBytes);
  float* o1 = (float*)c.dalloc(oBytes);
  GA_HIP(hipMemsetAsync(nr, 0, hBytes, c.stream));
  GA_HIP(hipMemsetAsync(ni, 0, hBytes, c.stream));
  GA_HIP(hipMemsetAsync(o0, 0, oBytes, c.stream));
  GA_HIP(hipMemsetAsync(o1, 0, oBytes, c.stream));
  if (g.rp > 0) {
    if (hist > 0 && !g.histZero) {
      GA_HIP(hipMemcpy2DAsync(nr, (size_t)need * 4, g.histR, (size_t)g.rp * 4, (size_t)g.rp * 4, (size_t)kBins * hist,
                              hipMemcpyDeviceToDevice, c.stream));
      GA_HIP(hipMemcpy2DAsync(ni, (size_t)need * 4, g.histI, (size_t)g.rp * 4, (size_t)g.rp * 4, (size_t)kBins * hist,
                              hipMemcpyDeviceToDevice, c.stream));
// ... 279 lines not shown
      pc.leader = leader;
      pc.ncol = w;
      for (int j = 0; j < w; j++) {
        pc.irCh[j] = cols[c0 + j][0];
        pc.outCh[j] = cols[c0 + j][1];
      }
      pieces.push_back(pc);
      c0 += w;
    }
  }
}

void CoarseStage::buildRows() {
  for (size_t di = 0; di < dNodes.size(); di++) {
    const int id = dNodes[di];
    NodeS& nd = *c.nodes[id];
    IrSpectra& ir = *nd.ir;
    const int P = ir.coarseP;
    if (P < 1 || P > kCoarseMaxP) fail(GA_ERR_INVALID_OPERATION, "internal: coarse partition count out of range");
    const int64_t hl = nd.dHistLen;
    GroupInfo& gi0 = groups[nd.dLeader >= 0 ? nd.dLeader : id];
    const bool carried = gi0.noHist;
    const Views& chIn = chInOf[di];
    const int nxr = nd.bShared ? 1 : nd.bInCh;
    c.stats.mac_flops_total += 8.0 * ir.P * kBins * (double)nd.bSlots * (double)n;
    c.stats.mac_bytes_total += ((double)ir.P * kBins * 8.0 + kBins * 8.0 + 512.0) * nd.bSlots * (double)n;
    if (gi0.premix) {
      for (int ch = 0; ch < nxr; ch++) {
        const float* oldHist = coarseHistory(nd, ch);
        float* nextHist = nd.dHist[nd.dHistCur ^ 1] + (size_t)ch * hl;
        PremixTerm t{chIn[ch], nullptr};
        if (coarseHistoryStays(c, nd, ch, chIn[ch], frames)) {
        } else if (c.coarseCarry && chIn[ch] && frames >= hl && ((uintptr_t)nextHist & 15) == 0) {
          t.carry = nextHist;
          pmBytes += (double)hl * 4.0;
        } else {
          hjobs.push_back(CoarseHistJob{oldHist, chIn[ch], nextHist, hl, frames});
          maxHist = std::max(maxHist, hl);
          histBytes += 2.0 * (double)hl * 4.0;
        }
        if (!gi0.terms) gi0.terms = std::make_unique<GroupInfo::Terms>();
        gi0.terms->in[ch].push_back(t);
        if (!carried) gi0.terms->hist[ch].push_back(PremixTerm{oldHist, nullptr});
      }
      nd.dHistCur ^= 1;
      nd.dHistZero = false;
      continue;
    }
    int xFrame[32], xIndex[32];
    for (int ch = 0; ch < nxr; ch++) {
      CoarseXRow r;
      const float* oldHist = coarseHistory(nd, ch);
      r.hist = carried ? nullptr : oldHist;
      r.in = chIn[ch];
      r.nvalid = frames;
      r.frame0 = frameNext;
      r.u0 = carried ? 0 : -(P - 1);
      r.n_frames = (gi0.tail ? nT + 1 : nT) - r.u0;
      r.hist_len = (int)hl;
      r.flags = 0;
      r.scale = 1.0f;
      xFrame[ch] = frameNext;
      xIndex[ch] = (int)xrows.size();
      frameNext += r.n_frames;
      float* nextHist = nd.dHist[nd.dHistCur ^ 1] + (size_t)ch * hl;
      r.carry = nullptr;
      r.carry_from = 0;
      if (coarseHistoryStays(c, nd, ch, r.in, frames)) {
      } else if (c.coarseCarry && r.in && frames >= hl && (((uintptr_t)r.in | (uintptr_t)nextHist) & 15) == 0) {
        r.carry = nextHist;
        r.carry_from = frames - hl;
        carryBytes[(int)xrows.size()] = (double)hl * 4.0;
      } else {
        hjobs.push_back(CoarseHistJob{oldHist, r.in, nextHist, hl, frames});
        maxHist = std::max(maxHist, hl);
        histBytes += 2.0 * (double)hl * 4.0;
      }
      xrows.push_back(r);
    }
    nd.dHistCur ^= 1;
    nd.dHistZero = false;
    addPieces(nd, nd.dLeader >= 0 ? nd.dLeader : id, nxr, xFrame, xIndex);
  }
  for (auto& kv : groups) {
    GroupInfo& g = kv.second;
    if (!g.premix) continue;
    NodeS& ld = *c.nodes[kv.first];
    const int64_t hl = g.hl0;
    int xFrame[32], xIndex[32];
    for (int ch = 0; ch < g.nxr; ch++) {
      const size_t bytes = (size_t)(hl + frames) * sizeof(float);
      if (pmUsed + bytes > c.coarseM.bytes) fail(GA_ERR_INVALID_OPERATION, "internal: the pre-mix arena is too small for the plan");
      float* mixed = (float*)((char*)c.coarseM.p + pmUsed);
      pmUsed += (bytes + 255) & ~(size_t)255;
      auto job = [&](float* out, const std::vector<PremixTerm>& tv, int64_t len, int64_t carryFrom) {
        PremixJob j{out, (int)pmTerms.size(), 0, len, carryFrom, 1, 0};
        for (const PremixTerm& t : tv) {
          if (!t.in) continue;
          pmTerms.push_back(t);
          j.nterms++;
          if ((uintptr_t)t.in & 15) j.flags &= ~1;
          if (t.carry) j.flags |= 2;
          pmBytes += (double)len * 4.0;
          pmFlops += (double)len * 4.0;
        }
        pmJobs.push_back(j);
        pmMaxN = std::max(pmMaxN, len);
        pmBytes += (double)len * 4.0;
      };
      if (!g.terms) g.terms = std::make_unique<GroupInfo::Terms>();
      if (!g.noHist) job(mixed, g.terms->hist[ch], hl, hl);
      job(mixed + hl, g.terms->in[ch], frames, std::max<int64_t>(0, frames - hl));
      CoarseXRow r{};
      r.hist = g.noHist ? nullptr : mixed;
      r.in = mixed + hl;
      r.nvalid = frames;
      r.frame0 = frameNext;
      r.u0 = g.noHist ? 0 : -(g.maxP - 1);
      r.n_frames = (g.tail ? nT + 1 : nT) - r.u0;
      r.hist_len = (int)hl;
      r.flags = 0;
      r.scale = 1.0f;
      r.carry = nullptr;
      r.carry_from = 0;
      xFrame[ch] = frameNext;
      xIndex[ch] = (int)xrows.size();
      frameNext += r.n_frames;
      xrows.push_back(r);
    }
    addPieces(ld, kv.first, g.nxr, xFrame, xIndex);
    c.stats.coarse_premixed_signals += (int64_t)g.members * g.nxr;
  }
  if (!pmJobs.empty() && !c.pendingHandOver.empty()) {
    std::vector<PremixJob> head;
    for (const Context::HandOver& h : c.pendingHandOver) {
      head.push_back(PremixJob{h.dst_dev, (int)pmTerms.size(), 1, h.n, h.n, 1 | 4, 0});
      pmTerms.push_back(PremixTerm{h.src, nullptr});
      pmMaxN = std::max(pmMaxN, h.n);
      pmBytes += 2.0 * (double)h.n * 4.0;
    }
    pmJobs.insert(pmJobs.begin(), head.begin(), head.end());
    c.pendingHandOver.clear();
    c.stats.deferred_handovers++;
  } else if (!c.pendingHandOver.empty() && !xrows.empty()) {
    for (const Context::HandOver& h : c.pendingHandOver) fwdHandOver.push_back(CoarseHandOver{h.src, h.dst_dev, h.n});
    c.pendingHandOver.clear();
    c.stats.deferred_handovers++;
  }
  ex.flushLevel();
}

void CoarseStage::buildJobs() {
  struct Key {
    int leader, P, ncol;
    std::array<int, 16> out;
    bool operator<(const Key& o) const { return std::tie(leader, P, ncol, out) < std::tie(o.leader, o.P, o.ncol, o.out); }
  };
  std::map<Key, std::vector<const Piece*>> byKey;
  for (const Piece& pc : pieces) {
    Key k{pc.leader, pc.P, pc.ncol, {}};
    k.out.fill(-1);
    for (int j = 0; j < pc.ncol; j++) k.out[j] = pc.outCh[j];
    byKey[k].push_back(&pc);
  }
  nxAll = (int)xrows.size();
  G = !c.coarseOverlap ? 1 : (nxAll >= 256 ? 4 : (nxAll >= 64 ? 2 : 1));
  auto groupOf = [&](int xrow) { return std::min(G - 1, (int)((int64_t)xrow * G / std::max(nxAll, 1))); };
  for (int g = 0; g <= G; g++) gBegin[g] = 0;
  for (int x = 0; x < nxAll; x++) gBegin[groupOf(x) + 1] = x + 1;
  for (int g = 1; g <= G; g++) gBegin[g] = std::max(gBegin[g], gBegin[g - 1]);
  for (auto& kv : byKey) {
    const Key& k = kv.first;
    const int cw = k.ncol, ci = cw == 1 ? 0 : (cw == 2 ? 1 : (cw == 4 ? 2 : 3));
    const auto& pv = kv.second;
    for (size_t p0 = 0; p0 < pv.size(); p0 += kVoicesPerJob) {
      const size_t p1 = std::min(pv.size(), p0 + kVoicesPerJob);
      const int term0 = (int)terms.size();
      bool shared = true;
      int lastX = 0;
      for (size_t i = p0; i < p1; i++) {
        const Piece& pc = *pv[i];
        CoarseTerm t{};
        t.frame0 = pc.frame0 - (pc.u0 + (pc.P - 1));
        for (int j = 0; j < 16; j++) t.h[j] = nullptr;
        for (int j = 0; j < cw; j++) t.h[j] = pc.ir->coarse + (size_t)pc.irCh[j] * pc.P * kCoarseBins;
        if (i > p0)
          for (int j = 0; j < cw; j++) shared = shared && (t.h[j] == terms[term0].h[j]);
        terms.push_back(t);
        lastX = std::max(lastX, pc.xrow);
      }
      if (cw == 16) {
        shared = false;
        for (size_t i = term0; i < terms.size(); i++)
          for (int j = 1; j < 16; j++) wideStrided = wideStrided && terms[i].h[j] == terms[i].h[0] + (size_t)j * k.P * kCoarseBins;
      }
      const int grp = groupOf(lastX);
      const int yrow0 = yNext;
      yNext += cw;
      for (int j = 0; j < cw; j++) outRows[{k.leader, k.out[j]}].push_back(yrow0 + j);
      const int jb = shared ? kCoarseSumJobBlocks(cw) : kCoarseJobBlocks(cw);
      const GroupInfo& gi = groups[k.leader];
      const int nTo = gi.tail ? nT + gi.maxP : nT;
      for (int t0 = 0; t0 < nTo; t0 += jb) {
        CoarseJob jb_{};
        jb_.term0 = term0;
        jb_.n_terms = (int)(p1 - p0);
        jb_.P = k.P;
        jb_.t0 = t0;
        jb_.n_t = std::min(jb, nTo - t0);
        jb_.yrow0 = yrow0;
        jb_.shared_h = shared ? 1 : 0;
        jb_.u_lo = gi.noHist ? 0 : -(k.P - 1);
        jb_.u_hi = gi.tail ? nT : nT - 1;
        const int cj = 2 * ci + (shared ? 1 : 0);
        jobs[cj][grp].push_back(jb_);
        maxT[cj] = std::max(maxT[cj], jb_.n_t);
        maxP[cj] = std::max(maxP[cj], k.P);
        while (k.P % pbOf[cj]) pbOf[cj] >>= 1;
        const int fread = std::max(0, std::min(jb_.u_hi, t0 + jb_.n_t - 1) - std::max(jb_.u_lo, t0 - (k.P - 1)) + 1);
        macBytes[cj][grp] += (double)jb_.n_terms * fread * kCoarseBins * 8.0 +
                             (t0 == 0 ? (double)(shared ? 1 : jb_.n_terms) * k.P * cw * kCoarseBins * 8.0 : 0.0) + (double)cw * jb_.n_t * kCoarseBins * 8.0;
        macFlops[cj][grp] += shared ? ((double)jb_.n_terms * fread * 2.0 + (double)k.P * jb_.n_t * cw * 8.0) * kCoarseBins
                                    : (double)jb_.n_terms * k.P * jb_.n_t * cw * 8.0 * kCoarseBins;
      }
    }
  }
}

void CoarseStage::buildOutputs() {
  int maxPAll = 0;
  for (auto& kv : groups)
    if (kv.second.tail) maxPAll = std::max(maxPAll, kv.second.maxP);
  yFrames = nT + maxPAll;
  invBlocks = nT;
  if (tails) {
    std::map<int, int> chOf;
    for (auto& kv : outRows) chOf[kv.first.first] = std::max(chOf[kv.first.first], kv.first.second + 1);
    for (auto& kv : groups) {
      if (!kv.second.tail) continue;
      NodeS& ld = *c.nodes[kv.first];
      const int64_t len = (int64_t)(kv.second.maxP + 1) * kCoarseBlock;
      const int nch = chOf.count(kv.first) ? chOf[kv.first] : 0;
      if (nch == 0) continue;
      if (!ld.dTail[0] || ld.dTailLen != len || ld.dTailCh != nch) {
        if (kv.second.carried) fail(GA_ERR_INVALID_OPERATION, "internal: a carried tail changed its shape");
        GA_HIP(hipStreamSynchronize(c.stream));
        for (int b = 0; b < 2; b++) {
          if (ld.dTail[b]) c.dfree(ld.dTail[b], (size_t)ld.dTailLen * ld.dTailCh * sizeof(float));
          ld.dTail[b] = (float*)c.dalloc((size_t)len * nch * sizeof(float));
        }
        ld.dTailLen = len;
        ld.dTailCh = nch;
        ld.dTailCur = 0;
      }
    }
  }
  for (auto& kv : outRows) {
    CoarseOut o{};
    o.out = ex.nodeOut(kv.first.first, kv.first.second);
    o.nvalid = frames;
    o.y0 = (int)ylist.size();
    o.ny = (int)kv.second.size();
    o.n_y = nT;
    if (groups[kv.first.first].tail) {
      NodeS& ld = *c.nodes[kv.first.first];
      const GroupInfo& gi = groups[kv.first.first];
      o.n_y = nT + gi.maxP;
      o.tail_len = ld.dTailLen;
      o.tail_in = gi.carried ? ld.dTail[ld.dTailCur] + (size_t)kv.first.second * ld.dTailLen : nullptr;
      o.tail_out = ld.dTail[ld.dTailCur ^ 1] + (size_t)kv.first.second * ld.dTailLen;
      invBlocks = std::max(invBlocks, (int)((frames + o.tail_len + kCoarseBlock - 1) / kCoarseBlock));
      invBytes += (double)o.tail_len * 4.0 * (gi.carried ? 2.0 : 1.0);
      if (gi.carried) c.stats.coarse_carried_outputs++;
    }
    ylist.insert(ylist.end(), kv.second.begin(), kv.second.end());
    outs.push_back(o);
    invBytes += (double)o.ny * o.n_y * kCoarseBins * 8.0 + (double)frames * 4.0;
    invFlops += (double)o.n_y * (kCoarseTransformFlops + (double)o.ny * 2.0 * kCoarseBins);
  }
  if (tails)
    for (auto& kv : groups) {
      NodeS& ld = *c.nodes[kv.first];
      if (!kv.second.tail || !ld.dTail[0]) continue;
      ld.dTailCur ^= 1;
      ld.dTailSig = kv.second.sig;
      ld.dTailSeq = c.chunkSeq;
    }
  if ((size_t)frameNext * kCoarseBins * sizeof(float2) > c.coarseX.bytes || (size_t)yNext * yFrames * kCoarseBins * sizeof(float2) > c.coarseY.bytes)
    fail(GA_ERR_INVALID_OPERATION, "internal: coarse spectra arenas are too small for the plan");

}

void CoarseStage::enqueue() {
  const int G = this->G, yFrames = this->yFrames, invBlocks = this->invBlocks, nxAll = this->nxAll;
  const double invBytes = this->invBytes, histBytes = this->histBytes;
  const size_t xo = ex.plan.putv(xrows), ho = ex.plan.putv(hjobs), to = ex.plan.putv(terms), oo = ex.plan.putv(outs), yo = ex.plan.putv(ylist);
  const size_t pjo = ex.plan.putv(pmJobs), pto = ex.plan.putv(pmTerms), fho = ex.plan.putv(fwdHandOver);
  const int nfh = (int)fwdHandOver.size();
  const int npm = (int)pmJobs.size();
  const int64_t pmMaxN = this->pmMaxN;
  const double pmBytes = this->pmBytes, pmFlops = this->pmFlops, invFlops = this->invFlops;
  struct MacLaunch { size_t off; int nj, cw, mt, mp, pb, grp; bool ap; double bytes, flops; };
  const bool matrixCores = c.coarseMfma && wideStrided;
  std::vector<MacLaunch> macs;
  for (int g = 0; g < G; g++)
    for (int i = 0; i < 8; i++) {
      if (jobs[i][g].empty()) continue;
      macs.push_back(MacLaunch{ex.plan.putv(jobs[i][g]), (int)jobs[i][g].size(), kCwOf[i >> 1], maxT[i], maxP[i], pbOf[i], g, (i & 1) == 0,
                               macBytes[i][g], macFlops[i][g]});
      c.stats.mac_launches += 1;
    }
  hipStream_t st = c.stream;
  float2* X = (float2*)c.coarseX.p;
  float2* Y = (float2*)c.coarseY.p;
  const float2* tw16 = c.twiddles16(4096);
  const float2* twFwd = c.twiddles16pw();
  const float2* twab = c.coarseTwab();
  const int nh = (int)hjobs.size(), no = (int)outs.size();
  struct FwdLaunch { int x0, nx, maxFrames, run; double bytes, flops; };
  std::vector<FwdLaunch> fwds;
  for (int g = 0; g < G; g++) {
    FwdLaunch f{this->gBegin[g], this->gBegin[g + 1] - this->gBegin[g], 0, 1, 0.0, 0.0};
    for (int x = f.x0; x < f.x0 + f.nx; x++) {
      f.maxFrames = std::max(f.maxFrames, xrows[x].n_frames);
      f.bytes += (double)(xrows[x].n_frames + 1) * kCoarseBlock * 4.0 + (double)xrows[x].n_frames * kCoarseBins * 8.0;
      f.flops += (double)xrows[x].n_frames * kCoarseTransformFlops;
      if (auto it = carryBytes.find(x); it != carryBytes.end()) f.bytes += it->second;
    }
    while (f.run < 16 && (int64_t)nxAll * ((f.maxFrames + 2 * f.run - 1) / (2 * f.run)) >= 1024) f.run *= 2;
    if (f.run >= 8) {
      const int k = (f.maxFrames + 11) / 12;
      f.run = (f.maxFrames + k - 1) / k;
    }
    if (const char* e = expenv("GA_COARSE_RUN")) f.run = std::max(1, atoi(e));
    fwds.push_back(f);
  }
  if (G > 1) c.ensureOverlapStream();
  Context* cp = &c;
  ex.plan.add(GA_STAGE_COARSE_SECTION, [=](uint8_t* base) {
    auto timed = [&](hipStream_t sx, int kind, double bytes, double flops, const std::function<const char*()>& launch) {
      hipEvent_t e0 = nullptr, e1 = nullptr;
      if (cp->profileNow) {
        GA_HIP(hipEventCreate(&e0));
        GA_HIP(hipEventCreate(&e1));
        GA_HIP(hipEventRecord(e0, sx));
      }
      cp->noteKernel(kind, launch());
      if (cp->profileNow) {
        GA_HIP(hipEventRecord(e1, sx));
        cp->extraProf.push_back(Context::ExtraProf{e0, e1, kind, bytes});
      }
      cp->stats.kernel_launches++;
      cp->stats.stage_launches[kind]++;
      cp->stats.stage_bytes[kind] += bytes;
      cp->stats.stage_flops[kind] += flops;
    };
    hipStream_t s2 = G > 1 ? cp->stream2 : st;
    if (npm > 0)
      timed(st, LK_CPREMIX, pmBytes, pmFlops, [&] { return launch_coarse_premix(st, (const PremixJob*)(base + pjo), npm, (const PremixTerm*)(base + pto), pmMaxN); });
    for (int g = 0; g < G; g++) {
      const FwdLaunch& f = fwds[g];
      if (f.nx > 0)
        timed(st, LK_CFWD, f.bytes, f.flops, [&] {
          return launch_coarse_fwd(st, (const CoarseXRow*)(base + xo) + f.x0, f.nx, f.maxFrames, f.run, X, twFwd, twab,
                                   (const CoarseHandOver*)(base + fho), g == 0 ? nfh : 0);
        });
      if (G > 1) {
        GA_HIP(hipEventRecord(cp->dGroupEv[g], st));
        GA_HIP(hipStreamWaitEvent(s2, cp->dGroupEv[g], 0));
      }
      for (const MacLaunch& m : macs)
        if (m.grp == g)
          timed(s2, LK_CMAC, m.bytes, m.flops, [&] {
            return launch_coarse_mac(s2, (const CoarseJob*)(base + m.off), m.nj, (const CoarseTerm*)(base + to), X, Y, yFrames, m.cw, m.mt, m.mp, m.ap, m.pb,
                                     matrixCores);
          });
    }
    if (G > 1) {
      GA_HIP(hipEventRecord(cp->dJoinEv, s2));
      GA_HIP(hipStreamWaitEvent(st, cp->dJoinEv, 0));
    }
  });
  ex.plan.add(LK_CINV, [=](uint8_t* base) {
    cp->noteKernel(LK_CINV, launch_coarse_inv(st, (const CoarseOut*)(base + oo), no, invBlocks, (const int*)(base + yo), Y, yFrames, tw16, twab));
  }, invBytes, invFlops);
  const int64_t mh = maxHist;
  if (nh > 0) ex.plan.add(LK_CHIST, [=](uint8_t* base) { launch_coarse_hist(st, (const CoarseHistJob*)(base + ho), nh, mh); }, histBytes);
}
}

static void planCoarseStage(Context& c, Exec& ex, const std::vector<int>& dNodes, int64_t n) {
  CoarseStage s(c, ex, dNodes, n);
  s.resolveInputs();
  s.classifyGroups();
  s.buildRows();
  s.buildJobs();
  s.buildOutputs();
  s.enqueue();
}

void Context::aliasBusToLeader(ChunkRun& r) {
  Exec& ex = *r.ex;
  int leader = -1, nch = 0;
  for (const Segment& sg : r.segs) {
    if (sg.nodes.empty() || sg.nodes.back().id != 0 || sg.nodes.back().ins.empty()) return;
    const InSeg& is = sg.nodes.back().ins[0];
    for (const TermS& t : is.terms) {
      const NodeS& nd = *nodes[t.node];
      if (nd.type != GA_NODE_CONVOLVER || !nd.ir || nd.convPath != 4 || nd.dLeader < 0 || t.out != 0 || t.ch != is.bufCh) return;
      if (leader < 0) {
        leader = nd.dLeader;
        nch = is.bufCh;
      } else if (leader != nd.dLeader || nch != is.bufCh) {
        return;
      }
    }
  }
  if (leader < 0 || nch < 1 || nch > (int)busSlabs.size()) return;
  const NodeS& ld = *nodes[leader];
  if (ld.outputs.empty() || ld.outputs[0].connectedInputs.size() != 1) return;
  const InRef& to = ld.outputs[0].connectedInputs[0];
  if (to.node != 0 || to.input != 0) return;
  for (int ch = 0; ch < nch; ch++) ex.setNodeOut(leader, ch, busTarget[ch] ? busTarget[ch] : busSlabs[ch]);
}

void Context::chunkConvScratch(ChunkRun& r) {
  Context& c_ = *this; (void)c_;
  std::vector<int>& topo = r.topo;
  int& maxDepth = r.maxDepth; int& maxLevel = r.maxLevel; (void)maxDepth; (void)maxLevel;
  int64_t& n = r.n; (void)n;
  std::vector<double>& bt = r.bt; (void)bt;
  std::vector<int>& srcIds = r.srcIds; (void)srcIds;
  std::vector<SrcPlanOut>& srcPlans = r.srcPlans; (void)srcPlans;
  std::vector<Segment>& segs = r.segs; (void)segs;
  const int64_t frames = r.n * kBlock; (void)frames;
  int& bHistMax = r.bHistMax; (void)bHistMax;
  for (auto& kv : resamplers) kv.second->devOffset = -1;

  if (topoHasConvolvers && r.stage != 1) {
    refOrderSensitivity(topo);
    assignConvPaths(topo, n);
    for (int id : topo) {
      NodeS& nd = *nodes[id];
      if (nd.type == GA_NODE_CONVOLVER) nd.refOrder = nd.refSens && nd.ir && (nd.convPath == 2 || nd.convPath == 3);
    }
    planCoarseFusion(topo, segs);
    for (int id : topo)
      if (nodes[id]->type == GA_NODE_CONVOLVER) nodes[id]->dGroupSize = 0;
    for (int id : topo) {
      const NodeS& nd = *nodes[id];
      if (nd.type == GA_NODE_CONVOLVER && nd.ir && nd.convPath == 4 && nd.dLeader >= 0) nodes[nd.dLeader]->dGroupSize++;
    }
    aliasBusToLeader(r);
  }
  bHistMax = 0;
  if (topoHasConvolvers) {
    size_t xMax = 0, yMax = 0;
    size_t bx = 0, by = 0;
    for (int id : topo) {
      NodeS& nd = *nodes[id];
      if (nd.type != GA_NODE_CONVOLVER || !nd.ir) continue;
      if (nd.convPath == 2 || nd.convPath == 3) {
        bx += nd.bInCh;
        by += nd.bSlots;
        bHistMax = std::max(bHistMax, nd.ir->P - 1);
      }
      for (auto& rr : nd.convRows) {
        ConvGroup& g = *rr.group;
        ensureGroupState(g);
        const int ty_ = (int)roundup(n, 64), tx_ = ty_ + g.P + 128;
        xMax = std::max(xMax, (size_t)kBins * tx_ * g.rp * sizeof(float));
        yMax = std::max(yMax, (size_t)kBins * ty_ * g.rp * sizeof(float));
      }
    }
    if (xMax) {
      ensure(planes[0], xMax);
      ensure(planes[1], xMax);
      ensure(planes[2], yMax);
      ensure(planes[3], yMax);
    }
    {
      std::map<int, std::pair<size_t, size_t>> perDepth;
      const int64_t nT = (n * kBlock + kCoarseBlock - 1) / kCoarseBlock;
      for (int id : topo) {
        NodeS& nd = *nodes[id];
        if (nd.type != GA_NODE_CONVOLVER || !nd.ir || nd.convPath != 4) continue;
        auto& pd = perDepth[nd.depth];
        pd.first += (size_t)nd.bInCh * (size_t)(nT + nd.ir->coarseP);
        pd.second += (size_t)nd.bSlots * (size_t)(nT + kCoarseMaxP);
      }
      size_t xf = 0, yf = 0;
      for (auto& kv : perDepth) {
        xf = std::max(xf, kv.second.first);
        yf = std::max(yf, kv.second.second);
      }
      if (xf) {
        ensure(coarseX, xf * kCoarseBins * sizeof(float2));
        ensure(coarseY, yf * kCoarseBins * sizeof(float2));
      }
      if (coarsePremix) {
        std::map<int, int> members;
        for (int id : topo) {
          NodeS& nd = *nodes[id];
          if (nd.type == GA_NODE_CONVOLVER && nd.ir && nd.convPath == 4) members[nd.dLeader >= 0 ? nd.dLeader : id]++;
        }
        std::map<int, size_t> pmDepth;
        for (auto& kv : members) {
          if (kv.second < 2) continue;
          const NodeS& ld = *nodes[kv.first];
          pmDepth[ld.depth] += (size_t)ld.bInCh * ((((size_t)(ld.dHistLen + n * kBlock) * sizeof(float)) + 255) & ~(size_t)255);
        }
        size_t pm = 0;
        for (auto& kv : pmDepth) pm = std::max(pm, kv.second);
        if (pm) ensure(coarseM, pm);
      }
    }
    bRowX = bRowY = 0;
    if (bx) {
      const size_t txb = (size_t)roundup(bHistMax, 4) + roundup(n, 16) + 16, tyb = (size_t)roundup(n, 256);
      bPairWrite = bPairCur ^ 1;
      flushPlaneHistories(bPairWrite);
      const size_t xb = bx * kBins * txb * sizeof(float);
      if (planesB[0].bytes < xb || planesBalt[0].bytes < xb) flushPlaneHistories(bPairCur);
      ensure(planesB[0], xb);
      ensure(planesB[1], xb);
      ensure(planesBalt[0], xb);
      ensure(planesBalt[1], xb);
      ensure(planesB[2], by * kBins * tyb * sizeof(float));
      ensure(planesB[3], by * kBins * tyb * sizeof(float));
    }
  }

  if (topoHasOscillators)
  for (int id : topo) {
    NodeS& nd = *nodes[id];
    if (nd.type != GA_NODE_OSCILLATOR || nd.oscPhase) continue;
    nd.oscPhase = (double*)dalloc(64);
    GA_HIP(hipMemsetAsync(nd.oscPhase, 0, 64, stream));
  }
}

void Context::planConvolversShared(ChunkRun& r, int d, ConvPlanCtx& k) {
  Context& c_ = *this; (void)c_;
  std::vector<int>& topo = r.topo;
  int& maxDepth = r.maxDepth; int& maxLevel = r.maxLevel; (void)maxDepth; (void)maxLevel;
  int64_t& n = r.n; (void)n;
  std::vector<double>& bt = r.bt; (void)bt;
  std::vector<int>& srcIds = r.srcIds; (void)srcIds;
  std::vector<SrcPlanOut>& srcPlans = r.srcPlans; (void)srcPlans;
  std::vector<Segment>& segs = r.segs; (void)segs;
  const int64_t frames = r.n * kBlock; (void)frames;
  int& bHistMax = r.bHistMax; (void)bHistMax;
  Exec& ex = *r.ex;
  (void)d; (void)topo;
  auto& active = k.active; auto& tsTemps = k.tsTemps; auto& prevIns = k.prevIns; int& prevP = k.prevP; int& prevRp = k.prevRp; int& prevRows = k.prevRows;
  for (auto& kv : active) {
    ConvGroup& g = *kv.first;
    const int P = g.P, hist = P - 1;
    const int nrows = (int)g.rows.size();
    std::vector<ConvRowIO> rio(nrows, ConvRowIO{nullptr, nullptr});
    for (auto& ns_ : kv.second) {
      NodeS& nd = *nodes[ns_.first];
      const int slot = ns_.second;
      const int idx = nd.convRows[slot].idx;
      const int inCh = nd.isTrueStereo ? (slot >> 1) : slot;
      const Exec::ConvInRow ci = ex.convIn[ns_.first];
      const float* stable = nullptr;
      bool same = true, first = true;
      for (size_t si = 0; si < segs.size(); si++) {
        const float* v = (ci[si].empty() || inCh >= (int)ci[si].size()) ? nullptr : ci[si][inCh];
        if (first) { stable = v; first = false; } else if (v != stable) same = false;
      }
      const float* in = stable;
      if (!same) {
        float* slab = getSlab(*this);
        for (size_t si = 0; si < segs.size(); si++) {
          const float* v = (ci[si].empty() || inCh >= (int)ci[si].size()) ? nullptr : ci[si][inCh];
          MixJob mj;
          mj.out = slab;
          mj.term0 = (int)ex.terms.size();
          mj.nterms = v ? 1 : 0;
          mj.f0 = segs[si].b0 * kBlock;
          mj.n = (segs[si].b1 - segs[si].b0) * kBlock;
          if (v) {
            ex.terms.push_back(v);
            ex.noteAlign(v, mj.f0);
          }
          ex.mixJobs.push_back(mj);
        }
        in = slab;
      }
      float* out;
      if (nd.isTrueStereo) {
        out = getSlab(*this);
      } else {
        out = ex.nodeOut(ns_.first, slot);
      }
// ... 368 lines not shown
```

### graphaudio_amd/csrc/ga_plan_nodes.cpp

```cpp
#include "ga_chunk_internal.hpp"

namespace ga {

void Context::chunkParamCurves(ChunkRun& r) {
  Context& c_ = *this; (void)c_;
  std::vector<int>& topo = r.topo;
  int& maxDepth = r.maxDepth; int& maxLevel = r.maxLevel; (void)maxDepth; (void)maxLevel;
  int64_t& n = r.n; (void)n;
  std::vector<double>& bt = r.bt; (void)bt;
  std::vector<int>& srcIds = r.srcIds; (void)srcIds;
  std::vector<SrcPlanOut>& srcPlans = r.srcPlans; (void)srcPlans;
  std::vector<Segment>& segs = r.segs; (void)segs;
  const int64_t frames = r.n * kBlock; (void)frames;
  int& bHistMax = r.bHistMax; (void)bHistMax;
  Exec& ex = *r.ex;
  {
    if (curveListEpoch != apiEpoch || curveListGraphVersion != graphVersion || curveListTopoSize != topo.size()) {
      for (auto& e : curveList)
        if (e.first < (int)nodes.size() && nodes[e.first] && e.second < (int)nodes[e.first]->params.size()) nodes[e.first]->params[e.second].curve = nullptr;
      curveList.clear();
      for (int id : topo) {
        NodeS& nd = *nodes[id];
        for (auto& p : nd.params) p.curve = nullptr;
        if (nd.type != GA_NODE_GAIN && nd.type != GA_NODE_BIQUAD && nd.type != GA_NODE_CONSTANT_SOURCE && nd.type != GA_NODE_OSCILLATOR &&
// ... 605 lines not shown
        fuseLen[b_.id] = la_ + 1;
      }
      int curLevel = -1, levelBqHeads = 0;
      if (d == 0 && topoHasCycles && cycleBlocks > 1) {
        for (const NodeSeg& ns : sg.nodes) {
          NodeS& nd = *nodes[ns.id];
          if (nd.type != GA_NODE_DELAY || !nd.delaySplit) continue;
          auto& ov = ex.outViews[si][ns.id];
          ov.assign(std::max(ns.outCh, 1), nullptr);
          NodePlanCtx k{r, ex, si, sg, f0, nf, nb, ns, nd, ov, segNode, absorbedBy, 0};
          k.delayPhase = 1;
          planDelay(k);
        }
        ex.flushLevel();
      }
      for (size_t ti = 0; ti < todo.size(); ti++) {
        const NodeSeg* nsp = todo[ti];
        if (ti + 4 < todo.size()) {
          const char* nx = (const char*)nodes[todo[ti + 4]->id].get();
          __builtin_prefetch(nx);
          __builtin_prefetch(nx + 64);
          __builtin_prefetch(nx + 128);
        }
        const NodeSeg& ns = *nsp;
        NodeS& nd = *nodes[ns.id];
        if (ns.level != curLevel) {
          ex.flushLevel();
          curLevel = ns.level;
          levelBqHeads = 0;
          for (size_t tj = ti; tj < todo.size() && todo[tj]->level == curLevel; tj++) {
            const NodeSeg& o = *todo[tj];
            if (o.type == GA_NODE_BIQUAD && o.bqActive && !o.bqDynamic && absorbedBy.get(o.id) < 0) levelBqHeads += std::max(o.outCh, 1);
          }
        }
        auto& ov = ex.outViews[si][ns.id];
        const bool cutDelay = nd.type == GA_NODE_DELAY && nd.delaySplit && topoHasCycles && cycleBlocks > 1;
        if (!cutDelay) ov.assign(nd.type == GA_NODE_CHANNEL_SPLITTER ? (int)nd.outputs.size() : std::max(ns.outCh, 1), nullptr);
        NodePlanCtx k{r, ex, si, sg, f0, nf, nb, ns, nd, ov, segNode, absorbedBy, levelBqHeads};
        if (cutDelay) k.delayPhase = 2;
        switch (nd.type) {
          case GA_NODE_CHANNEL_SPLITTER: {
            if (!ns.outMask) break;
            auto iv = ex.resolveInput((int)si, ns, 0, false, nullptr);
            for (int o = 0; o < (int)nd.outputs.size(); o++)
              if ((ns.outMask >> o) & 1) ov[o] = iv[o];
            break;
          }
          case GA_NODE_CHANNEL_MERGER: {
            for (int i = 0; i < (int)ns.ins.size(); i++) {
              if (!((ns.outMask >> i) & 1)) continue;
              auto iv = ex.resolveInput((int)si, ns, i, false, nullptr);
              ov[i] = iv.empty() ? nullptr : iv[0];
            }
            break;
          }
          case GA_NODE_CONSTANT_SOURCE: planConstantSource(k); break;
          case GA_NODE_OSCILLATOR: planOscillator(k); break;
          case GA_NODE_DELAY: planDelay(k); break;
          case GA_NODE_STEREO_PANNER: planStereoPanner(k); break;
          case GA_NODE_BUFFER_SOURCE: planBufferSource(k); break;
          case GA_NODE_STREAM_SOURCE: planStreamSource(k); break;
          case GA_NODE_GAIN: planGain(k); break;
          case GA_NODE_BIQUAD: planBiquad(k); break;
          case GA_NODE_CONVOLVER: {
            auto iv = ex.resolveInput((int)si, ns, 0, false, nullptr);
            if (!nd.ir) break;
            ex.convIn[ns.id][si] = iv;
            if (nd.convPath == 4 && nd.dLeader >= 0 && nd.dLeader != ns.id) break;
#ifdef GA_EXPERIMENTS
            static const bool noZeroPage = getenv("GA_NO_ZERO_PAGE") != nullptr;
#else
            constexpr bool noZeroPage = false;
#endif
            if (!noZeroPage && ns.outZero && !(nd.convPath == 4 && nd.dGroupSize > 1)) {
              for (int ch = 0; ch < ns.outCh; ch++) ov[ch] = zeros;
              break;
            }
            for (int ch = 0; ch < ns.outCh; ch++) ov[ch] = ex.nodeOut(ns.id, ch);
            break;
          }
          case GA_NODE_DESTINATION: {
            SmallVec<float*, 4> forced((size_t)std::max(ns.ins[0].bufCh, 1), nullptr);
            for (int ch = 0; ch < ns.ins[0].bufCh && ch < (int)busSlabs.size(); ch++) forced[ch] = busTarget[ch] ? busTarget[ch] : busSlabs[ch];
            ex.resolveInput((int)si, ns, 0, true, forced.data());
            break;
          }
          default: break;
        }
      }
      ex.flushLevel();
    }
}

void Context::chunkStaleSeed(ChunkRun& r) {
  if (staleProducers.empty() && staleLeavers.empty()) return;
  Exec& ex = *r.ex;
  std::vector<StaleJob> jobs;
  auto alive = [&](const float* p) {
    if (!p) return false;
    const size_t blockBytes = (size_t)slabFrames * sizeof(float) * std::max<size_t>(8, std::min<size_t>(1024, ((size_t)1 << 30) / std::max<size_t>((size_t)slabFrames * sizeof(float), 1)));
    for (void* b : slabBlocks)
      if ((const char*)p >= (const char*)b && (const char*)p + kBlock * sizeof(float) <= (const char*)b + blockBytes) return true;
    for (const auto& np : nodes) {
      const NodeS& o = *np;
      if (o.staleBuf && p >= o.staleBuf && p + kBlock <= o.staleBuf + (size_t)o.staleRows * kBlock) return true;
      if (o.staleNext && p >= o.staleNext && p + kBlock <= o.staleNext + (size_t)o.staleRows * kBlock) return true;
    }
    return false;
  };
  const bool haveLast = lastViewSlabGen == slabGen && lastViewFrames >= kBlock;
  auto keepLastBlock = [&](NodeS& nd) {
    const int id = nd.id;
    const int rows = nd.type == GA_NODE_CHANNEL_SPLITTER ? std::max<int>(1, (int)nd.outputs.size()) : 32;
    if (!nd.staleBuf) {
      nd.staleRows = rows;
      nd.staleBuf = (float*)dalloc((size_t)rows * kBlock * sizeof(float));
      nd.staleNext = (float*)dalloc((size_t)rows * kBlock * sizeof(float));
      GA_HIP(hipMemsetAsync(nd.staleNext, 0, (size_t)rows * kBlock * sizeof(float), stream));
    }
    const bool haveViews = haveLast && id < (int)lastViews.size();
    const float g = (haveViews && id < (int)lastViewScale.size()) ? lastViewScale[id] : 1.f;
    const float* cv = (haveViews && id < (int)lastViewCurve.size() && lastViewCurve[id]) ? lastViewCurve[id] + (lastViewFrames - kBlock) : nullptr;
    for (int rw = 0; rw < nd.staleRows; rw++) {
      const float* src = (haveViews && rw < (int)lastViews[id].size() && lastViews[id][rw]) ? lastViews[id][rw] + (lastViewFrames - kBlock) : nullptr;
      StaleJob sj{nd.staleBuf + (size_t)rw * kBlock, alive(src) ? src : nullptr, g, 0};
      sj.curve = (sj.src && cv && alive(cv)) ? cv : nullptr;
      jobs.push_back(sj);
#ifdef GA_EXPERIMENTS
      if (expenv("GA_DEBUG_STALE") && rw < 2)
        fprintf(stderr, "[stale] chunk %llu node %d type %d row %d: views %d (of %zu nodes) view %p alive %d scale %g curve %p\n", (unsigned long long)chunkSeq, id,
                nd.type, rw, haveViews ? (int)lastViews[id].size() : -1, lastViews.size(), (const void*)src, (int)alive(src), g, (const void*)sj.curve);
#endif
    }
  };
  for (int id : staleProducers) {
    NodeS& nd = *nodes[id];
    if (nd.staleBuf && nd.staleSeq + 1 == chunkSeq) continue;
    if (nd.prevReachable || !nd.staleBuf) keepLastBlock(nd);
  }
  for (int id : staleLeavers) {
    NodeS& nd = *nodes[id];
    if (nd.staleBuf && nd.staleSeq + 1 == chunkSeq) continue;
    if (!haveLast || id >= (int)lastViews.size()) continue;
    bool any = false;
    for (const float* v : lastViews[id]) any = any || v != nullptr;
    if (any || nd.staleBuf) keepLastBlock(nd);
  }
  staleLeavers.clear();
  if (jobs.empty()) return;
  const size_t off = ex.plan.putv(jobs);
  const int nj = (int)jobs.size();
  hipStream_t st = stream;
  ex.plan.add(LK_OTHER, [=](uint8_t* base) { launch_stale_copy(st, (const StaleJob*)(base + off), nj); });
}

void Context::chunkStaleCommit(ChunkRun& r) {
  if (staleProducers.empty()) return;
  Exec& ex = *r.ex;
  std::vector<StaleJob> jobs;
  const int si = (int)r.segs.size() - 1;
  for (int id : staleProducers) {
    NodeS& nd = *nodes[id];
    const int rows = nd.type == GA_NODE_CHANNEL_SPLITTER ? std::max<int>(1, (int)nd.outputs.size()) : 32;
    if (!nd.staleBuf || nd.staleRows < rows) {
      if (nd.staleBuf) {
        GA_HIP(hipStreamSynchronize(stream));
        dfree(nd.staleBuf, (size_t)nd.staleRows * kBlock * sizeof(float));
// ... 52 lines not shown
```

Measured before the change: 1.247 billion.

## Batch deferred coarse convolution tails across several render chunks

Adds a tail-batch mode: for qualifying single-stage coarse convolver chunks rendered with deferred host hand-over, the forward FFT, MAC and inverse stages are postponed and later flushed together for several chunks in one set of launches. A chain kernel adds the carried tails between consecutive chunks. To make this work it grows the spectra and pre-mix arenas, the deferred staging slots and the per-node tail buffers. The aim is to amortize launch and small-grid overhead across chunks. It brings substantial bookkeeping and many flush points, and it is gated by a new option 'coarse_tail_batch' whose default appears to be 1, which leaves the feature off.

```diff
diff --git a/graphaudio_amd/csrc/ga_api.cpp b/graphaudio_amd/csrc/ga_api.cpp
--- a/graphaudio_amd/csrc/ga_api.cpp
+++ b/graphaudio_amd/csrc/ga_api.cpp
@@ -52,6 +52,10 @@
 template <class F>
 int guard(ga_context* h, F&& f) {
   if (h) h->c.apiEpoch++;
+  if (h && !h->c.pendingTails.empty()) {
+    const int rc = guardRO(h, [](Context& c) { c.flushTails("an API call that edits the context"); });
+    if (rc != GA_OK) return rc;
+  }
   return guardRO(h, std::forward<F>(f));
 }
 NodeS* typed(Context& c, int id, int type) {
@@ -228,28 +232,55 @@
     }
     struct Target {
       Context& c;
-      ~Target() { std::memset(c.busTarget, 0, sizeof(c.busTarget)); }
+      ~Target() {
+        std::memset(c.busTarget, 0, sizeof(c.busTarget));
+        c.tailArmed = false;
+      }
     } target{*this};
     const bool defer = direct && !deviceOut && pipelined.callerAsync && hostDefer && ownStream;
+    if (!defer) {
+      flushTails("a render whose bus is not deferred");
+      if (!pendingHandOver.empty() && pendingHandOver.front().id != pendingHandOver.back().id) flushHandOver();
+    }
+    tailArmed = defer && tailBatch > 1;
     if (defer) {
       const size_t rowBytes = ((size_t)nblk * kBlock * sizeof(float) + 255) & ~(size_t)255;
-      if (deferStageBytes < rowBytes * 32) {
+      const int slots = tailBatch > 1 ? 2 * tailBatch : 1;
+      const int rows = tailBatch > 1 ? std::max(channels, 2) : 32;
+      if (deferStageBytes < rowBytes * rows * slots || deferSlots != slots || deferRows < rows) {
         flushHandOver();
         if (deferStage) {
           GA_HIP(hipStreamSynchronize(stream));
           dfree(deferStage, deferStageBytes);
         }
-        deferStageBytes = rowBytes * 32;
+        deferSlots = slots;
+        deferRows = rows;
+        deferStageBytes = rowBytes * rows * slots;
         deferStage = (float*)dalloc(deferStageBytes);
       }
-      for (int ch = 0; ch < channels; ch++) busTarget[ch] = (float*)((char*)deferStage + (size_t)ch * (deferStageBytes / 32));
+      const size_t slotBytes = deferStageBytes / deferSlots, rowStride = (slotBytes / deferRows) & ~(size_t)255;
+      const char* slot0 = (const char*)deferStage + (size_t)(deferSlotSeq++ % deferSlots) * slotBytes;
+      if (deferSlots > 1) {
+        bool busy = false;
+        for (const HandOver& h : pendingHandOver) busy = busy || ((const char*)h.src >= slot0 && (const char*)h.src < slot0 + slotBytes);
+        for (const PendingTail& t : pendingTails)
+          for (const CoarseOut& o : t.outs) busy = busy || ((const char*)o.out >= slot0 && (const char*)o.out < slot0 + slotBytes);
+        if (busy) flushHandOver();
+      }
+      for (int ch = 0; ch < channels; ch++) busTarget[ch] = (float*)(slot0 + (size_t)ch * rowStride);
     } else if (direct) {
       for (int ch = 0; ch < channels; ch++) busTarget[ch] = tgt[ch];
     }
     runChunk(nblk, nullptr);
-    if (defer)
+    if (defer) {
+      std::vector<HandOver>& q = lastChunkDeferred && !pendingTails.empty() ? pendingTails.back().handOver : pendingHandOver;
+      const uint64_t id = ++handOverSeq;
       for (int ch = 0; ch < channels; ch++)
-        pendingHandOver.push_back(HandOver{busTarget[ch], tgt[ch], out[ch] + startIndex + written, chunkBlocksDone * kBlock});
+        q.push_back(HandOver{busTarget[ch], tgt[ch], out[ch] + startIndex + written, chunkBlocksDone * kBlock, id});
+      if (lastChunkDeferred && (int)pendingTails.size() >= tailBatch) flushTails("the batch is full");
+    }
+    lastChunkDeferred = false;
+    tailArmed = false;
     std::memset(busTarget, 0, sizeof(busTarget));
     const int64_t done = chunkBlocksDone;
     if (done <= 0) fail(GA_ERR_INVALID_OPERATION, "render made no progress");
@@ -361,6 +392,7 @@
     else if (k == "conv_reference_order") c.convRefOrder = (int)std::min(2.0, std::max(0.0, value));
     else if (k == "conv_ref_min_deviation") c.convRefMinDeviation = std::max(0.0, value);
     else if (k == "coarse_premix") c.coarsePremix = value != 0;
+    else if (k == "coarse_tail_batch") c.tailBatch = (int)std::min<double>(Context::kMaxTailBatch, std::max(1.0, value));
     else if (k == "coarse_ext_history") c.coarseExtHist = value != 0;
     else if (k == "coarse_wide") c.coarseWide = value != 0;
     else if (k == "gain_pass_through") c.gainPassThrough = value != 0;
diff --git a/graphaudio_amd/csrc/ga_chunk.cpp b/graphaudio_amd/csrc/ga_chunk.cpp
--- a/graphaudio_amd/csrc/ga_chunk.cpp
+++ b/graphaudio_amd/csrc/ga_chunk.cpp
@@ -614,7 +614,22 @@
   int& bHistMax = r.bHistMax; (void)bHistMax;
   Exec& ex = *r.ex;
   r.tmPlan = nowMs();
-  if (!pendingHandOver.empty()) {
+  bool deferTail = false;
+  if (ex.tailCand && tailArmed && asyncMode && tailBatch > 1 && r.stage == 0 && ex.coarseStages == 1 && !ex.busWritten) {
+    const PendingTail& t = *ex.tailCand;
+    if (!pendingTails.empty()) {
+      const PendingTail& p = pendingTails.front();
+      if (p.frames != t.frames || p.xFrames != t.xFrames || p.yRows != t.yRows || p.yFrames != t.yFrames || p.invBlocks != t.invBlocks ||
+          p.fwdRun != t.fwdRun || p.fwdMaxFrames != t.fwdMaxFrames || (int)pendingTails.size() >= tailBatch)
+        flushTails("the chunks' shape changes");
+    }
+    const size_t members = pendingTails.size() + 1;
+    deferTail = members * (size_t)t.xFrames * kCoarseBins * sizeof(float2) <= coarseX.bytes &&
+                members * (size_t)t.yRows * t.yFrames * kCoarseBins * sizeof(float2) <= coarseY.bytes;
+  }
+  if (!deferTail && !pendingTails.empty()) flushTails("a chunk that does not qualify");
+  lastChunkDeferred = false;
+  if (!pendingHandOver.empty() && !handOverTaken) {
     std::vector<HandOver> hv;
     hv.swap(pendingHandOver);
     hipStream_t st = stream;
@@ -652,7 +667,13 @@
     GA_HIP(hipEventCreate(&evEnd));
     GA_HIP(hipEventRecord(evBegin, stream));
   }
+  struct DeferNow {
+    bool& f;
+    ~DeferNow() { f = false; }
+  } deferNow{tailDeferNow};
+  tailDeferNow = deferTail;
   for (auto& l : ex.plan.launches) {
+    if (deferTail && l.kind == LK_CINV) continue;
     hipEvent_t e0 = nullptr, e1 = nullptr;
     if (profile) {
       GA_HIP(hipEventCreate(&e0));
@@ -682,6 +703,13 @@
   extraProf.clear();
   if (profile) GA_HIP(hipEventRecord(evEnd, stream));
   GA_HIP(hipGetLastError());
+  tailDeferNow = false;
+  if (deferTail) {
+    ex.tailCand->profiled = profile;
+    pendingTails.push_back(std::move(*ex.tailCand));
+    ex.tailCand.reset();
+    lastChunkDeferred = true;
+  }
   r.tmLaunch = nowMs();
   if (profileNow) pendingProf.push_back(ProfBatch{evBegin, evEnd, std::move(evs), std::move(evKind), std::move(evBytes)});
   if (asyncMode) {
@@ -700,6 +728,148 @@
     fprintf(stderr, "[ga] chunk %lld blocks: sim %.2f ms, plan %.2f ms, enqueue %.2f ms, wait %.2f ms\n", (long long)n, r.tmSim - r.tm0,
             r.tmPlan - r.tmSim, r.tmLaunch - r.tmPlan, nowMs() - r.tmLaunch);
 
+}
+
+void Context::flushTails(const char* why) {
+  if (pendingTails.empty()) return;
+  std::vector<PendingTail> batch;
+  batch.swap(pendingTails);
+  const double t0 = nowMs();
+  const int m = (int)batch.size();
+  GA_HIP(hipSetDevice(device));
+  Plan tb;
+  std::vector<CoarseXRow> xrows;
+  std::vector<CoarseTerm> terms;
+  std::vector<CoarseJob> jobs[6];
+  std::vector<CoarseOut> outs;
+  std::vector<int> ylist;
+  std::vector<CoarseChain> chain;
+  int maxT[6] = {}, maxP[6] = {}, pbOf[6] = {4, 4, 4, 4, 4, 4};
+  double macBytes[6] = {}, macFlops[6] = {}, fwdBytes = 0, fwdFlops = 0, invBytes = 0, invFlops = 0;
+  int64_t chainMax = 0;
+  int nprof = 0;
+  const PendingTail& p0 = batch.front();
+  if ((size_t)m * p0.xFrames * kCoarseBins * sizeof(float2) > coarseX.bytes || (size_t)m * p0.yRows * p0.yFrames * kCoarseBins * sizeof(float2) > coarseY.bytes)
+    fail(GA_ERR_INVALID_OPERATION, "internal: coarse spectra arenas are too small for a batch of deferred stages");
+  for (int k = 0; k < m; k++) {
+    PendingTail& t = batch[k];
+    const int xBase = k * p0.xFrames, yBase = k * p0.yRows, termBase = (int)terms.size(), ylBase = (int)ylist.size();
+    for (CoarseXRow r : t.xrows) {
+      r.frame0 += xBase;
+      xrows.push_back(r);
+    }
+    for (CoarseTerm tm : t.terms) {
+      tm.frame0 += xBase;
+      terms.push_back(tm);
+    }
+    for (int i = 0; i < 6; i++) {
+      for (CoarseJob j : t.jobs[i]) {
+        j.term0 += termBase;
+        j.yrow0 += yBase;
+        jobs[i].push_back(j);
+      }
+      if (t.jobs[i].empty()) continue;
+      maxT[i] = std::max(maxT[i], t.maxT[i]);
+      maxP[i] = std::max(maxP[i], t.maxP[i]);
+      pbOf[i] = std::min(pbOf[i], t.pbOf[i]);
+      macBytes[i] += t.macBytes[i];
+      macFlops[i] += t.macFlops[i];
+    }
+    for (CoarseOut o : t.outs) {
+      o.y0 += ylBase;
+      if (k > 0 && o.tail_in) {
+        chain.push_back(CoarseChain{o.out, o.tail_in, o.tail_len});
+        chainMax = std::max(chainMax, o.tail_len);
+        o.tail_in = nullptr;
+      }
+      outs.push_back(o);
+    }
+    for (int y : t.ylist) ylist.push_back(y + yBase);
+    fwdBytes += t.fwdBytes;
+    fwdFlops += t.fwdFlops;
+    invBytes += t.invBytes;
+    invFlops += t.invFlops;
+    nprof += t.profiled ? 1 : 0;
+  }
+  const size_t xo = tb.putv(xrows), to = tb.putv(terms), oo = tb.putv(outs), yo = tb.putv(ylist), co = tb.putv(chain);
+  size_t jo[6];
+  for (int i = 0; i < 6; i++) jo[i] = tb.putv(jobs[i]);
+  const size_t tbytes = (tb.host.size() + 15) & ~(size_t)15;
+  const int hs = (int)(tailFlushSeq++ % kTailStage);
+  if (tailHostDone[hs]) GA_HIP(hipEventSynchronize(tailHostDone[hs]));
+  if (tailHostBytes[hs] < tbytes) {
+    if (tailHost[hs]) (void)hipHostFree(tailHost[hs]);
+    tailHost[hs] = nullptr;
+    tailHostBytes[hs] = (tbytes + tbytes / 4 + 4096 + 15) & ~(size_t)15;
+    GA_HIP(hipHostMalloc(&tailHost[hs], tailHostBytes[hs], hipHostMallocDefault));
+  }
+  ensure(tailTables, tbytes + tbytes / 4 + 4096);
+  std::memset(tailHost[hs], 0, tbytes);
+  std::memcpy(tailHost[hs], tb.host.data(), tb.host.size());
+  if (tableUploadKernel) launch_table_upload(stream, tailTables.p, tailHost[hs], tbytes);
+  else GA_HIP(hipMemcpyAsync(tailTables.p, tailHost[hs], tbytes, hipMemcpyHostToDevice, stream));
+  if (!tailHostDone[hs]) GA_HIP(hipEventCreateWithFlags(&tailHostDone[hs], hipEventDisableTiming));
+  GA_HIP(hipEventRecord(tailHostDone[hs], stream));
+  uint8_t* base = (uint8_t*)tailTables.p;
+  hipStream_t st = stream;
+  float2* X = (float2*)coarseX.p;
+  float2* Y = (float2*)coarseY.p;
+  ProfBatch pb{};
+  pb.tailBatch = true;
+  pb.share = (double)nprof / (double)m;
+  const bool prof = nprof > 0;
+  if (prof) {
+    GA_HIP(hipEventCreate(&pb.begin));
+    GA_HIP(hipEventCreate(&pb.end));
+    GA_HIP(hipEventRecord(pb.begin, st));
+  }
+  auto timed = [&](int kind, double bytes, double flops, const std::function<const char*()>& launch) {
+    hipEvent_t e0 = nullptr, e1 = nullptr;
+    if (prof) {
+      GA_HIP(hipEventCreate(&e0));
+      GA_HIP(hipEventCreate(&e1));
+      GA_HIP(hipEventRecord(e0, st));
+    }
+    noteKernel(kind, launch());
+    if (prof) {
+      GA_HIP(hipEventRecord(e1, st));
+      pb.evs.push_back({e0, e1});
+      pb.kinds.push_back(kind);
+      pb.bytes.push_back(bytes);
+    }
+    stats.kernel_launches++;
+    stats.stage_launches[kind]++;
+    stats.stage_bytes[kind] += bytes;
+    stats.stage_flops[kind] += flops;
+  };
+  static constexpr int kCw[3] = {1, 2, 4};
+  timed(LK_CFWD, fwdBytes, fwdFlops, [&] {
+    return launch_coarse_fwd(st, (const CoarseXRow*)(base + xo), (int)xrows.size(), p0.fwdMaxFrames, p0.fwdRun, X, twiddles16pw(), coarseTwab());
+  });
+  for (int i = 0; i < 6; i++) {
+    if (jobs[i].empty()) continue;
+    timed(LK_CMAC, macBytes[i], macFlops[i], [&] {
+      stats.mac_launches += 1;
+      return launch_coarse_mac(st, (const CoarseJob*)(base + jo[i]), (int)jobs[i].size(), (const CoarseTerm*)(base + to), X, Y, p0.yFrames, kCw[i >> 1], maxT[i],
+                               maxP[i], (i & 1) == 0, pbOf[i], false);
+    });
+  }
+  timed(LK_CINV, invBytes, invFlops, [&] {
+    return launch_coarse_inv(st, (const CoarseOut*)(base + oo), (int)outs.size(), p0.invBlocks, (const int*)(base + yo), Y, p0.yFrames, twiddles16(4096), coarseTwab());
+  });
+  if (!chain.empty()) {
+    launch_coarse_chain(st, (const CoarseChain*)(base + co), (int)chain.size(), chainMax);
+    stats.kernel_launches++;
+    stats.stage_launches[LK_OTHER]++;
+  }
+  if (prof) {
+    GA_HIP(hipEventRecord(pb.end, st));
+    pendingProf.push_back(std::move(pb));
+  }
+  GA_HIP(hipGetLastError());
+  for (PendingTail& t : batch)
+    for (const HandOver& h : t.handOver) pendingHandOver.push_back(h);
+  if (gaTiming) fprintf(stderr, "[ga] tail batch: %d chunks flushed (%s), enqueue %.3f ms\n", m, why ? why : "", nowMs() - t0);
 }
 
 void Context::chunkCommit(ChunkRun& r) {
@@ -790,6 +960,8 @@
   r.tm0 = nowMs();
   GA_HIP(hipSetDevice(device));
   if (disposed) fail(GA_ERR_DISPOSED, "context disposed");
+  handOverTaken = false;
+  if (!pendingTails.empty() && (!pending.empty() || !releasedPending.empty() || chunksSinceGc + 1 >= 64)) flushTails("queued commands");
   drain();
   if (!releasedPending.empty() || ++chunksSinceGc >= 64) collectGarbage();
   latched = true;
diff --git a/graphaudio_amd/csrc/ga_chunk_internal.hpp b/graphaudio_amd/csrc/ga_chunk_internal.hpp
--- a/graphaudio_amd/csrc/ga_chunk_internal.hpp
+++ b/graphaudio_amd/csrc/ga_chunk_internal.hpp
@@ -457,6 +457,9 @@
   Context& c;
   int64_t n, frames;
   Plan plan;
+  std::unique_ptr<Context::PendingTail> tailCand;
+  int coarseStages = 0;
+  bool busWritten = false;
   std::vector<Segment>& segs;
   std::unordered_map<uint64_t, float*> nodeSlab, inSlab;
   std::vector<float*> nodeSlab01;
diff --git a/graphaudio_amd/csrc/ga_coarse.hip b/graphaudio_amd/csrc/ga_coarse.hip
--- a/graphaudio_amd/csrc/ga_coarse.hip
+++ b/graphaudio_amd/csrc/ga_coarse.hip
@@ -1101,6 +1101,28 @@
     hipLaunchKernelGGL(coarse_hist_kernel, dim3(gx, std::min(32768, njobs - j0)), dim3(256), 0, s, jobs_dev + j0);
 }
 
+__global__ __launch_bounds__(256) void coarse_chain_kernel(const CoarseChain* __restrict jobs) {
+  const CoarseChain J = jobs[blockIdx.y];
+  if (((((uintptr_t)J.out | (uintptr_t)J.tail)) & 15) == 0) {
+    for (int64_t i = 4 * ((int64_t)blockIdx.x * blockDim.x + threadIdx.x); i < J.n; i += 4 * (int64_t)gridDim.x * blockDim.x) {
+      v4f v = *reinterpret_cast<const v4f*>(J.out + i);
+      v += ldg4(J.tail + i);
+      stg4(J.out + i, v);
+    }
+    return;
+  }
+  for (int64_t i = (int64_t)blockIdx.x * blockDim.x + threadIdx.x; i < J.n; i += (int64_t)gridDim.x * blockDim.x) {
+    float v = J.out[i];
+    v += ldg1(J.tail + i);
+    stg1(J.out + i, v);
+  }
+}
+void launch_coarse_chain(hipStream_t s, const CoarseChain* jobs_dev, int njobs, int64_t max_len) {
+  if (njobs <= 0 || max_len <= 0) return;
+  const int gx = (int)std::min<int64_t>((max_len / 4 + 255) / 256, 64);
+  hipLaunchKernelGGL(coarse_chain_kernel, dim3(gx, std::min(32768, njobs)), dim3(256), 0, s, jobs_dev);
+}
+
 __global__ __launch_bounds__(256) void table_upload_kernel(v4f* __restrict dst, const v4f* __restrict src, size_t n16) {
   for (size_t i = (size_t)blockIdx.x * 256 + threadIdx.x; i < n16; i += (size_t)gridDim.x * 256) ((GA_GLOBAL v4f*)dst)[i] = ((const GA_GLOBAL v4f*)src)[i];
 }
diff --git a/graphaudio_amd/csrc/ga_comm.cpp b/graphaudio_amd/csrc/ga_comm.cpp
--- a/graphaudio_amd/csrc/ga_comm.cpp
+++ b/graphaudio_amd/csrc/ga_comm.cpp
@@ -214,7 +214,8 @@
         }
       }
       if (locked) {
-        for (int ch = 0; ch < channels; ch++) pendingHandOver.push_back(HandOver{rows[ch], devAlias[ch], out[ch] + start, frames});
+        const uint64_t id = ++handOverSeq;
+        for (int ch = 0; ch < channels; ch++) pendingHandOver.push_back(HandOver{rows[ch], devAlias[ch], out[ch] + start, frames, id});
       } else if (callerAsync && ownStream && hostCopyStream) {
         handOverToHost(rows, out, channels, start, frames);
       } else {
diff --git a/graphaudio_amd/csrc/ga_engine.cpp b/graphaudio_amd/csrc/ga_engine.cpp
--- a/graphaudio_amd/csrc/ga_engine.cpp
+++ b/graphaudio_amd/csrc/ga_engine.cpp
@@ -217,8 +217,8 @@
     if (np && np->bOverlap) (void)hipFree(np->bOverlap);
     if (np && np->dHistBase[0]) (void)hipFree(np->dHistBase[0]);
     if (np && np->dHistBase[1]) (void)hipFree(np->dHistBase[1]);
-    if (np && np->dTail[0]) (void)hipFree(np->dTail[0]);
-    if (np && np->dTail[1]) (void)hipFree(np->dTail[1]);
+    for (int b = 0; np && b < NodeS::kTailBufs; b++)
+      if (np->dTail[b]) (void)hipFree(np->dTail[b]);
     if (np && np->stWin[0]) (void)hipFree(np->stWin[0]);
     if (np && np->stWin[1]) (void)hipFree(np->stWin[1]);
     if (np && np->delayHist) (void)hipFree(np->delayHist);
@@ -252,6 +252,11 @@
   if (coarseY.p) (void)hipFree(coarseY.p);
   if (coarseM.p) (void)hipFree(coarseM.p);
   if (deferStage) (void)hipFree(deferStage);
+  if (tailTables.p) (void)hipFree(tailTables.p);
+  for (int k = 0; k < kTailStage; k++) {
+    if (tailHost[k]) (void)hipHostFree(tailHost[k]);
+    if (tailHostDone[k]) (void)hipEventDestroy(tailHostDone[k]);
+  }
   for (auto& r : retired) (void)hipFree(r.first);
   for (auto& kv : resamplers)
     if (kv.second->devSamples) (void)hipFree(kv.second->devSamples);
@@ -377,10 +382,11 @@
     else if (hipEventQuery(b.end) != hipSuccess) { (void)hipGetLastError(); break; }
     float ms = 0;
     GA_HIP(hipEventElapsedTime(&ms, b.begin, b.end));
-    stats.device_ms_total += ms;
-    stats.profiled_chunks++;
+    stats.device_ms_total += ms * b.share;
+    if (!b.tailBatch) stats.profiled_chunks++;
     for (size_t i = 0; i < b.evs.size(); i++) {
       GA_HIP(hipEventElapsedTime(&ms, b.evs[i].first, b.evs[i].second));
+      ms *= (float)b.share;
       const int k = b.kinds[i];
       if (k == LK_MAC || k == LK_CMAC) stats.mac_ms_total += ms;
       else if (k == LK_FFT || k == LK_IFFT || k == LK_CFWD || k == LK_CINV || k == LK_CHIST) stats.fft_ms_total += ms;
@@ -394,7 +400,34 @@
     pendingProf.pop_front();
   }
 }
+std::vector<Context::HandOver> Context::takeHandOvers() {
+  std::vector<HandOver> out;
+  size_t i = 0;
+  int buses = 0;
+  while (i < pendingHandOver.size()) {
+    size_t j = i;
+    while (j < pendingHandOver.size() && pendingHandOver[j].id == pendingHandOver[i].id) j++;
+    bool clash = false;
+    for (size_t k = i; k < j && !clash; k++)
+      for (const HandOver& o : out) {
+        const float *a0 = pendingHandOver[k].dst_host, *a1 = a0 + pendingHandOver[k].n, *b0 = o.dst_host, *b1 = b0 + o.n;
+        if (a0 < b1 && b0 < a1) {
+          clash = true;
+          break;
+        }
+      }
+    if (clash) break;
+    out.insert(out.end(), pendingHandOver.begin() + (ptrdiff_t)i, pendingHandOver.begin() + (ptrdiff_t)j);
+    buses++;
+    i = j;
+  }
+  pendingHandOver.erase(pendingHandOver.begin(), pendingHandOver.begin() + (ptrdiff_t)i);
+  stats.deferred_handovers += buses;
+  handOverTaken = handOverTaken || buses > 0;
+  return out;
+}
 void Context::flushHandOver() {
+  flushTails("the buses are handed over");
   for (const HandOver& h : pendingHandOver)
     GA_HIP(hipMemcpyAsync(h.dst_host, h.src, sizeof(float) * (size_t)h.n, hipMemcpyDeviceToHost, stream));
   pendingHandOver.clear();
@@ -572,9 +605,10 @@
   }
   if (n.dTail[0]) {
     if (stream) (void)hipStreamSynchronize(stream);
-    for (int b = 0; b < 2; b++) dfree(n.dTail[b], (size_t)n.dTailLen * n.dTailCh * sizeof(float));
-  }
-  n.dTail[0] = n.dTail[1] = nullptr;
+    for (int b = 0; b < NodeS::kTailBufs; b++) dfree(n.dTail[b], (size_t)n.dTailLen * n.dTailCh * sizeof(float));
+  }
+  for (int b = 0; b < NodeS::kTailBufs; b++) n.dTail[b] = nullptr;
+  n.dTailN = 0;
   n.dTailLen = 0;
   n.dTailCh = n.dTailCur = 0;
   n.dTailSig = 0;
diff --git a/graphaudio_amd/csrc/ga_engine.hpp b/graphaudio_amd/csrc/ga_engine.hpp
--- a/graphaudio_amd/csrc/ga_engine.hpp
+++ b/graphaudio_amd/csrc/ga_engine.hpp
@@ -225,7 +225,9 @@
   int dHistCur = 0;
   bool dHistZero = true;
   bool everFed = false;
-  float* dTail[2] = {nullptr, nullptr};
+  static constexpr int kTailBufs = 5;
+  float* dTail[kTailBufs] = {nullptr, nullptr, nullptr, nullptr, nullptr};
+  int dTailN = 0;
   int64_t dTailLen = 0;
   int dTailCh = 0, dTailCur = 0;
   uint64_t dTailSig = 0, dTailSeq = ~0ull - 1;
@@ -511,6 +513,8 @@
     std::vector<std::pair<hipEvent_t, hipEvent_t>> evs;
     std::vector<int> kinds;
     std::vector<double> bytes;
+    double share = 1.0;
+    bool tailBatch = false;
   };
   std::deque<ProfBatch> pendingProf;
   void harvestProfile(bool wait);
@@ -693,8 +697,41 @@
 
   int64_t busCapFrames = 0;
   std::vector<float*> busSlabs;
-  struct HandOver { const float* src; float* dst_dev; float* dst_host; int64_t n; };
+  struct HandOver { const float* src; float* dst_dev; float* dst_host; int64_t n; uint64_t id = 0; };
   std::vector<HandOver> pendingHandOver;
+  uint64_t handOverSeq = 0;
+  bool handOverTaken = false;
+  std::vector<HandOver> takeHandOvers();
+  struct PendingTail {
+    int64_t frames = 0;
+    int xFrames = 0, yRows = 0, yFrames = 0, invBlocks = 0, fwdMaxFrames = 0, fwdRun = 1;
+    std::vector<CoarseXRow> xrows;
+    std::vector<CoarseTerm> terms;
+    std::vector<CoarseJob> jobs[6];
+    int maxT[6] = {}, maxP[6] = {}, pbOf[6] = {};
+    double macBytes[6] = {}, macFlops[6] = {};
+    std::vector<CoarseOut> outs;
+    std::vector<int> ylist;
+    double fwdBytes = 0, fwdFlops = 0, invBytes = 0, invFlops = 0;
+    std::vector<HandOver> handOver;
+    bool profiled = false;
+  };
+  static constexpr int kMaxTailBatch = 4;
+  int tailBatch = 1;
+  bool tailArmed = false;
+  bool tailDeferNow = false;
+  bool lastChunkDeferred = false;
+  uint64_t tailSlotSeq = 0;
+  uint64_t deferSlotSeq = 0;
+  int deferSlots = 0, deferRows = 0;
+  std::vector<PendingTail> pendingTails;
+  DevArena tailTables;
+  static constexpr int kTailStage = 4;
+  void* tailHost[kTailStage] = {nullptr, nullptr, nullptr, nullptr};
+  size_t tailHostBytes[kTailStage] = {0, 0, 0, 0};
+  hipEvent_t tailHostDone[kTailStage] = {nullptr, nullptr, nullptr, nullptr};
+  uint64_t tailFlushSeq = 0;
+  void flushTails(const char* why);
   std::vector<std::pair<void*, size_t>> retired;
   void freeRetired();
   float* deferStage = nullptr;
diff --git a/graphaudio_amd/csrc/ga_kernels.hpp b/graphaudio_amd/csrc/ga_kernels.hpp
--- a/graphaudio_amd/csrc/ga_kernels.hpp
+++ b/graphaudio_amd/csrc/ga_kernels.hpp
@@ -170,6 +170,12 @@
 const char* launch_coarse_inv(hipStream_t s, const CoarseOut* outs_dev, int nouts, int n_t, const int* ylist_dev, const float2* Y, int y_frames,
                        const float2* tw16, const float2* twab);
 void launch_coarse_hist(hipStream_t s, const CoarseHistJob* jobs_dev, int njobs, int64_t max_len);
+struct CoarseChain {
+  float* out;
+  const float* tail;
+  int64_t n;
+};
+void launch_coarse_chain(hipStream_t s, const CoarseChain* jobs_dev, int njobs, int64_t max_len);
 void launch_table_upload(hipStream_t s, void* dst, const void* src_pinned, size_t bytes);
 
 struct MixJob {
diff --git a/graphaudio_amd/csrc/ga_plan_conv.cpp b/graphaudio_amd/csrc/ga_plan_conv.cpp
--- a/graphaudio_amd/csrc/ga_plan_conv.cpp
+++ b/graphaudio_amd/csrc/ga_plan_conv.cpp
@@ -385,6 +385,9 @@
     nd.dHistZero = false;
     addPieces(nd, nd.dLeader >= 0 ? nd.dLeader : id, nxr, xFrame, xIndex);
   }
+  const int pmSlots = c.tailArmed && c.tailBatch > 1 ? c.tailBatch : 1;
+  const size_t pmSlotBytes = (c.coarseM.bytes / pmSlots) & ~(size_t)255;
+  const size_t pmSlotBase = (size_t)(c.tailSlotSeq % pmSlots) * pmSlotBytes;
   for (auto& kv : groups) {
     GroupInfo& g = kv.second;
     if (!g.premix) continue;
@@ -393,8 +396,8 @@
     int xFrame[32], xIndex[32];
     for (int ch = 0; ch < g.nxr; ch++) {
       const size_t bytes = (size_t)(hl + frames) * sizeof(float);
-      if (pmUsed + bytes > c.coarseM.bytes) fail(GA_ERR_INVALID_OPERATION, "internal: the pre-mix arena is too small for the plan");
-      float* mixed = (float*)((char*)c.coarseM.p + pmUsed);
+      if (pmUsed + bytes > pmSlotBytes) fail(GA_ERR_INVALID_OPERATION, "internal: the pre-mix arena is too small for the plan");
+      float* mixed = (float*)((char*)c.coarseM.p + pmSlotBase + pmUsed);
       pmUsed += (bytes + 255) & ~(size_t)255;
       auto job = [&](float* out, const std::vector<PremixTerm>& tv, int64_t len, int64_t carryFrom) {
         PremixJob j{out, (int)pmTerms.size(), 0, len, carryFrom, 1, 0};
@@ -436,19 +439,15 @@
   }
   if (!pmJobs.empty() && !c.pendingHandOver.empty()) {
     std::vector<PremixJob> head;
-    for (const Context::HandOver& h : c.pendingHandOver) {
+    for (const Context::HandOver& h : c.takeHandOvers()) {
       head.push_back(PremixJob{h.dst_dev, (int)pmTerms.size(), 1, h.n, h.n, 1 | 4, 0});
       pmTerms.push_back(PremixTerm{h.src, nullptr});
       pmMaxN = std::max(pmMaxN, h.n);
       pmBytes += 2.0 * (double)h.n * 4.0;
     }
     pmJobs.insert(pmJobs.begin(), head.begin(), head.end());
-    c.pendingHandOver.clear();
-    c.stats.deferred_handovers++;
   } else if (!c.pendingHandOver.empty() && !xrows.empty()) {
-    for (const Context::HandOver& h : c.pendingHandOver) fwdHandOver.push_back(CoarseHandOver{h.src, h.dst_dev, h.n});
-    c.pendingHandOver.clear();
-    c.stats.deferred_handovers++;
+    for (const Context::HandOver& h : c.takeHandOvers()) fwdHandOver.push_back(CoarseHandOver{h.src, h.dst_dev, h.n});
   }
   ex.flushLevel();
 }
@@ -547,11 +546,14 @@
       if (nch == 0) continue;
       if (!ld.dTail[0] || ld.dTailLen != len || ld.dTailCh != nch) {
         if (kv.second.carried) fail(GA_ERR_INVALID_OPERATION, "internal: a carried tail changed its shape");
+        if (!c.pendingTails.empty()) c.flushTails("a group's tail buffers change");
         GA_HIP(hipStreamSynchronize(c.stream));
-        for (int b = 0; b < 2; b++) {
+        for (int b = 0; b < NodeS::kTailBufs; b++) {
           if (ld.dTail[b]) c.dfree(ld.dTail[b], (size_t)ld.dTailLen * ld.dTailCh * sizeof(float));
-          ld.dTail[b] = (float*)c.dalloc((size_t)len * nch * sizeof(float));
+          ld.dTail[b] = nullptr;
         }
+        ld.dTailN = c.tailBatch > 1 ? std::min(c.tailBatch, Context::kMaxTailBatch) + 1 : 2;
+        for (int b = 0; b < ld.dTailN; b++) ld.dTail[b] = (float*)c.dalloc((size_t)len * nch * sizeof(float));
         ld.dTailLen = len;
         ld.dTailCh = nch;
         ld.dTailCur = 0;
@@ -571,7 +573,7 @@
       o.n_y = nT + gi.maxP;
       o.tail_len = ld.dTailLen;
       o.tail_in = gi.carried ? ld.dTail[ld.dTailCur] + (size_t)kv.first.second * ld.dTailLen : nullptr;
-      o.tail_out = ld.dTail[ld.dTailCur ^ 1] + (size_t)kv.first.second * ld.dTailLen;
+      o.tail_out = ld.dTail[(ld.dTailCur + 1) % ld.dTailN] + (size_t)kv.first.second * ld.dTailLen;
       invBlocks = std::max(invBlocks, (int)((frames + o.tail_len + kCoarseBlock - 1) / kCoarseBlock));
       invBytes += (double)o.tail_len * 4.0 * (gi.carried ? 2.0 : 1.0);
       if (gi.carried) c.stats.coarse_carried_outputs++;
@@ -585,7 +587,7 @@
     for (auto& kv : groups) {
       NodeS& ld = *c.nodes[kv.first];
       if (!kv.second.tail || !ld.dTail[0]) continue;
-      ld.dTailCur ^= 1;
+      ld.dTailCur = (ld.dTailCur + 1) % ld.dTailN;
       ld.dTailSig = kv.second.sig;
       ld.dTailSeq = c.chunkSeq;
     }
@@ -611,7 +613,6 @@
       if (jobs[i][g].empty()) continue;
       macs.push_back(MacLaunch{ex.plan.putv(jobs[i][g]), (int)jobs[i][g].size(), kCwOf[i >> 1], maxT[i], maxP[i], pbOf[i], g, (i & 1) == 0,
                                macBytes[i][g], macFlops[i][g]});
-      c.stats.mac_launches += 1;
     }
   hipStream_t st = c.stream;
   float2* X = (float2*)c.coarseX.p;
@@ -640,6 +641,47 @@
   }
   if (G > 1) c.ensureOverlapStream();
   Context* cp = &c;
+  ex.coarseStages++;
+  ex.tailCand.reset();
+  if (c.tailArmed && c.tailBatch > 1 && ex.coarseStages == 1 && ex.segs.size() == 1 && G == 1 && npm > 0 && nfh == 0 && !outs.empty() &&
+      jobs[6][0].empty() && jobs[7][0].empty()) {
+    bool ok = true;
+    for (auto& kv : groups) ok = ok && kv.second.premix && kv.second.tail && (int64_t)(kv.second.maxP + 1) * kCoarseBlock <= frames;
+    for (const CoarseOut& o : outs) {
+      bool bus = false;
+      for (int ch = 0; ch < 32; ch++) bus = bus || (c.busTarget[ch] && o.out == c.busTarget[ch]);
+      ok = ok && bus && o.tail_out && o.tail_len <= o.nvalid && o.nvalid == frames;
+    }
+    for (auto& kv : groups) ok = ok && c.nodes[kv.first]->dTailN >= c.tailBatch + 1;
+    if (ok) {
+      auto t = std::make_unique<Context::PendingTail>();
+      t->frames = frames;
+      t->xFrames = frameNext;
+      t->yRows = yNext;
+      t->yFrames = yFrames;
+      t->invBlocks = invBlocks;
+      t->fwdMaxFrames = fwds[0].maxFrames;
+      t->fwdRun = fwds[0].run;
+      t->fwdBytes = fwds[0].bytes;
+      t->fwdFlops = fwds[0].flops;
+      t->xrows = xrows;
+      t->terms = terms;
+      for (int i = 0; i < 6; i++) {
+        t->jobs[i] = jobs[i][0];
+        t->maxT[i] = maxT[i];
+        t->maxP[i] = maxP[i];
+        t->pbOf[i] = pbOf[i];
+        t->macBytes[i] = macBytes[i][0];
+        t->macFlops[i] = macFlops[i][0];
+      }
+      t->outs = outs;
+      t->ylist = ylist;
+      t->invBytes = invBytes;
+      t->invFlops = invFlops;
+      ex.tailCand = std::move(t);
+    }
+  }
+  if (npm > 0) c.tailSlotSeq++;
   ex.plan.add(GA_STAGE_COARSE_SECTION, [=](uint8_t* base) {
     auto timed = [&](hipStream_t sx, int kind, double bytes, double flops, const std::function<const char*()>& launch) {
       hipEvent_t e0 = nullptr, e1 = nullptr;
@@ -661,6 +703,7 @@
     hipStream_t s2 = G > 1 ? cp->stream2 : st;
     if (npm > 0)
       timed(st, LK_CPREMIX, pmBytes, pmFlops, [&] { return launch_coarse_premix(st, (const PremixJob*)(base + pjo), npm, (const PremixTerm*)(base + pto), pmMaxN); });
+    if (cp->tailDeferNow) return;
     for (int g = 0; g < G; g++) {
       const FwdLaunch& f = fwds[g];
       if (f.nx > 0)
@@ -675,6 +718,7 @@
       for (const MacLaunch& m : macs)
         if (m.grp == g)
           timed(s2, LK_CMAC, m.bytes, m.flops, [&] {
+            cp->stats.mac_launches += 1;
             return launch_coarse_mac(s2, (const CoarseJob*)(base + m.off), m.nj, (const CoarseTerm*)(base + to), X, Y, yFrames, m.cw, m.mt, m.mp, m.ap, m.pb,
                                      matrixCores);
           });
@@ -685,6 +729,7 @@
     }
   });
   ex.plan.add(LK_CINV, [=](uint8_t* base) {
+    if (cp->tailDeferNow) return;
     cp->noteKernel(LK_CINV, launch_coarse_inv(st, (const CoarseOut*)(base + oo), no, invBlocks, (const int*)(base + yo), Y, yFrames, tw16, twab));
   }, invBytes, invFlops);
   const int64_t mh = maxHist;
@@ -797,9 +842,10 @@
         xf = std::max(xf, kv.second.first);
         yf = std::max(yf, kv.second.second);
       }
+      const size_t batch = tailArmed && tailBatch > 1 ? (size_t)tailBatch : 1;
       if (xf) {
-        ensure(coarseX, xf * kCoarseBins * sizeof(float2));
-        ensure(coarseY, yf * kCoarseBins * sizeof(float2));
+        ensure(coarseX, batch * xf * kCoarseBins * sizeof(float2));
+        ensure(coarseY, batch * yf * kCoarseBins * sizeof(float2));
       }
       if (coarsePremix) {
         std::map<int, int> members;
@@ -815,7 +861,10 @@
         }
         size_t pm = 0;
         for (auto& kv : pmDepth) pm = std::max(pm, kv.second);
-        if (pm) ensure(coarseM, pm);
+        if (pm) {
+          if (coarseM.bytes < batch * pm && !pendingTails.empty()) flushTails("the pre-mix arena grows");
+          ensure(coarseM, batch * pm);
+        }
       }
     }
     bRowX = bRowY = 0;
diff --git a/graphaudio_amd/csrc/ga_plan_nodes.cpp b/graphaudio_amd/csrc/ga_plan_nodes.cpp
--- a/graphaudio_amd/csrc/ga_plan_nodes.cpp
+++ b/graphaudio_amd/csrc/ga_plan_nodes.cpp
@@ -711,7 +711,9 @@
           case GA_NODE_DESTINATION: {
             SmallVec<float*, 4> forced((size_t)std::max(ns.ins[0].bufCh, 1), nullptr);
             for (int ch = 0; ch < ns.ins[0].bufCh && ch < (int)busSlabs.size(); ch++) forced[ch] = busTarget[ch] ? busTarget[ch] : busSlabs[ch];
+            const size_t jobsBefore = ex.mixJobs.size();
             ex.resolveInput((int)si, ns, 0, true, forced.data());
+            if (ex.mixJobs.size() != jobsBefore) ex.busWritten = true;
             break;
           }
           default: break;
```

Result: slower. 1.234 billion, median of 2 (-1.0%).
